# GLAD-RUC/FastEGNN

Measured on AMD Instinct MI355X. Metric: graphs/sec (fwd+bwd), Water-3D-like 100k-node frame, higher is better.
Workload: dtype f32; 1 GPU; cfg4 Water-3D-like frame (SURVEY 8d): uniform points, radius graph r=0.035 (mean degree ~19), gravity on; 4-layer FastEGNN H=64, fwd+loss+bwd, CSR build inside the step; nodes=100000, edges=1919172, graphs_per_batch=1, virtual_channels=16, layers=4, parallelism=1 GPU, launch=whole step replayed as one captured HIP graph

## Files before the change

### fastegnn_amd/csrc/layer_bwd.hip

```cpp
#include "stages.h"
#ifdef FE_DIAG_NOSTORE
#define WG_STORE(x)
#else
#define WG_STORE(x) x
#endif

namespace fe {

__device__ __forceinline__ Vec vdsilu_mul(const Vec &g, const Vec &z FE_ACT_P) {
  return vmap2(g, z, [=](float a, float b) { return a * dsilu_f(b FE_ACT_A); });
}
__device__ __forceinline__ Vec vmask(const Vec &v, bool keep) { return keep ? v : vzero(); }

__device__ __forceinline__ void vec_reduce_lds(float *red_row, const Vec &acc, int j, int q) {
#pragma unroll
  for (int t = 0; t < 4; ++t)
#pragma unroll
    for (int r = 0; r < 4; ++r) {
      float s = jsum(acc.t[t][r]);
      if (j == 0) atomicAdd(&red_row[16 * t + 4 * q + r], s);
    }
}

struct GraphPostBwdArgs {
  const float *xsum, *HvT, *poolV, *g_Z_out, *g_HvT_out, *wpack, *b5;
  float *g_Z, *g_HvT, *g_poolV, *g_poolX, *wg_u, *wg_gz5, *wg_pm;
  int B, C, flags;
  float act_param = 0.f;
};
__global__ __launch_bounds__(256) void graph_post_bwd_kernel(GraphPostBwdArgs a) {
  const bool bf = a.flags & FASTEGNN_F_BF16;
  auto rb = [&](const Vec &v) { return bf ? vround(v) : v; };
  const int l = lane_id(), j = l & 15, q = l >> 4;
  const int wave = global_wave_id(), nwaves = (gridDim.x * blockDim.x) >> 6;
  const int M = a.B * a.C, ntiles = (M + 15) >> 4;
  for (int i = blockIdx.x * blockDim.x + threadIdx.x; i < a.B * 3 * a.C; i += gridDim.x * blockDim.x) {
    const int b = i / (3 * a.C);
    const float g = a.g_Z_out[i];
    a.g_Z[i] = g;
    a.g_poolX[i] = g / fmaxf(a.xsum[b * 4 + 3], 1.f);
  }
  if (a.flags & FASTEGNN_F_RF) {
    for (int i = blockIdx.x * blockDim.x + threadIdx.x; i < M * H; i += gridDim.x * blockDim.x) {
      a.g_HvT[i] = a.g_HvT_out[i];
      a.g_poolV[i] = 0.f;
    }
    return;
  }
  for (int tile = wave; tile < ntiles; tile += nwaves) {
    const int m = tile * 16 + j;
    const bool valid = m < M;
    const int mc = valid ? m : M - 1;
    const int b = mc / a.C;
    const float inv = 1.0f / fmaxf(a.xsum[b * 4 + 3], 1.f);
    const Vec hv = vload_row(a.HvT + (size_t)mc * H, q);
    const Vec pm = vscale(vload_row(a.poolV + (size_t)mc * H, q), inv);
    Vec z5 = vload_vec(a.b5, q);
    gemm64(a.wpack + (size_t)I_W5A * IMG, rb(hv), z5);
    gemm64(a.wpack + (size_t)I_W5B * IMG, rb(pm), z5);
    const Vec g_out = vload_row(a.g_HvT_out + (size_t)mc * H, q);
    Vec g_u = vzero();
    gemm64(a.wpack + (size_t)I_W6T * IMG, rb(g_out), g_u);
    const Vec g_z5 = vdsilu_mul(g_u, z5 FE_ACT(a));
    Vec g_hv = (a.flags & FASTEGNN_F_RESIDUAL) ? g_out : vzero();
    gemm64(a.wpack + (size_t)I_W5AT * IMG, rb(g_z5), g_hv);
    Vec g_pm = vzero();
    gemm64(a.wpack + (size_t)I_W5BT * IMG, rb(g_z5), g_pm);
    if (valid) {
      vstore_row(a.wg_u + (size_t)m * H, q, vsilu(z5 FE_ACT(a)));
      vstore_row(a.wg_gz5 + (size_t)m * H, q, g_z5);
      vstore_row(a.wg_pm + (size_t)m * H, q, pm);
      vstore_row(a.g_HvT + (size_t)m * H, q, g_hv);
      vstore_row(a.g_poolV + (size_t)m * H, q, vscale(g_pm, inv));
    }
  }
}

int graph_post_backward(const fastegnn_layer_t *L, hipStream_t st, WgradBatch *shared) {
  FE_REQUIRE(L->xsum && L->HvT && L->poolV && L->g_Z_out && L->g_HvT_out && L->g_Z && L->g_HvT && L->g_poolV &&
                 L->g_poolX && L->wg_node && L->grads && L->wpack,
             "graph_post_backward: null buffer");
  const long M = (long)L->B * L->C;
  float *wg_gp = L->wg_node + 4 * wg_node_rows(L) * H;
  float *wg_u = wg_gp, *wg_gz5 = wg_gp + M * H, *wg_pm = wg_gp + 2 * M * H;
  GraphPostBwdArgs a{L->xsum, L->HvT, L->poolV, L->g_Z_out, L->g_HvT_out, L->wpack, L->params[FASTEGNN_P_NODEV0_B],
                     L->g_Z, L->g_HvT, L->g_poolV, L->g_poolX, wg_u, wg_gz5, wg_pm, L->B, L->C, L->flags, L->act_param};
  int grid = cdiv(cdiv(M, 16), 4);
  if (grid > 256) grid = 256;
  if (grid < 1) grid = 1;
  { ProfScope _ps_graph_post_bwd_kernel(K_GRAPH_POST_BWD, st); hipLaunchKernelGGL(graph_post_bwd_kernel, dim3(grid), dim3(256), 0, st, a); }
  int rc = check_launch("graph_post_bwd_kernel");
  if (rc) return rc;
  if (has(L, FASTEGNN_F_RF)) return FASTEGNN_OK;
  float *const *g = L->grads;
  WgradBatch local(L->wg_slab, st);
  WgradBatch &wb = shared ? *shared : local;
  wb.round = has(L, FASTEGNN_F_BF16);
  if ((rc = wb.add(L->g_HvT_out, H, wg_u, H, M, g[FASTEGNN_P_NODEV2_W], H, 0, 1, g[FASTEGNN_P_NODEV2_B]))) return rc;
  if ((rc = wb.add(wg_gz5, H, L->HvT, H, M, g[FASTEGNN_P_NODEV0_W], 2 * H, 0, 1, g[FASTEGNN_P_NODEV0_B]))) return rc;
  if ((rc = wb.add(wg_gz5, H, wg_pm, H, M, g[FASTEGNN_P_NODEV0_W], 2 * H, H, 1, nullptr))) return rc;
  return shared ? FASTEGNN_OK : wb.finish();
}


struct GraphPreBwdArgs {
  const float *xsum, *Z, *g_Bc, *g_Zp, *V0W;
  float *g_Z, *g_HvT, *g_xbar, *wg_mxt;
  int B, C, bf16;
};
constexpr int GPB_SPLIT = 4;
__global__ __launch_bounds__(256) void graph_pre_bwd_kernel(GraphPreBwdArgs a) {
  extern __shared__ float sm[];
  const int C = a.C, b = blockIdx.x, ld = 2 * H + 1 + C;
  const int i0 = blockIdx.y * 256 + threadIdx.x, istep = 256 * gridDim.y;
  float *mz = sm;
  float *gmX = sm + 3 * C;
  float *gmz = gmX + C * C;
  const float cnt = fmaxf(a.xsum[b * 4 + 3], 1.f);
  for (int i = threadIdx.x; i < 3 * C; i += 256) mz[i] = a.Z[(size_t)b * 3 * C + i] - a.xsum[b * 4 + i / C] / cnt;
  __syncthreads();
  for (int i = i0; i < C * H; i += istep) {
    int c = i >> 6, d = i & 63;
    float v = 0.f;
    if (d < C) v = mz[c] * mz[d] + mz[C + c] * mz[C + d] + mz[2 * C + c] * mz[2 * C + d];
    a.wg_mxt[((size_t)b * C + c) * H + d] = v;
  }
  for (int i = i0; i < C * H; i += istep) {
    int c = i >> 6, k = i & 63;
    const float *gb = a.g_Bc + ((size_t)b * C + c) * H;
    float acc = 0.f;
    if (a.bf16) { for (int o = 0; o < H; ++o) acc += round_bf(gb[o]) * round_bf(a.V0W[(size_t)o * ld + H + k]); }
    else { for (int o = 0; o < H; ++o) acc += gb[o] * a.V0W[(size_t)o * ld + H + k]; }
    a.g_HvT[((size_t)b * C + c) * H + k] += acc;
  }
  for (int i = threadIdx.x; i < C * C; i += 256) {
    int cp = i / C, c = i % C;
    const float *gb = a.g_Bc + ((size_t)b * C + c) * H;
    float acc = 0.f;
    for (int o = 0; o < H; ++o) acc += gb[o] * a.V0W[(size_t)o * ld + 2 * H + 1 + cp];
    gmX[cp * C + c] = acc;
  }
  __syncthreads();
  for (int i = threadIdx.x; i < 3 * C; i += 256) {
    int k = i / C, c = i % C;
    float acc = 0.f;
    for (int d = 0; d < C; ++d) acc += (gmX[c * C + d] + gmX[d * C + c]) * mz[k * C + d];
    gmz[i] = acc;
    if (i % gridDim.y == blockIdx.y) a.g_Z[(size_t)b * 3 * C + i] += acc + a.g_Zp[(size_t)b * 3 * C + i];
  }
  __syncthreads();
  if (threadIdx.x < 3 && blockIdx.y == 0) {
    float acc = 0.f;
    for (int c = 0; c < C; ++c) acc += gmz[threadIdx.x * C + c];
    a.g_xbar[b * 3 + threadIdx.x] = -acc / cnt;
  }
}
int graph_pre_backward(const fastegnn_layer_t *L, hipStream_t st, WgradBatch *shared) {
  FE_REQUIRE(L->xsum && L->Z && L->HvT && L->g_Bc && L->g_Zp && L->g_Z && L->g_HvT && L->g_xbar && L->wg_node && L->grads,
             "graph_pre_backward: null buffer");
  const long M = (long)L->B * L->C;
  float *wg_mxt = L->wg_node + 7 * wg_node_rows(L) * H;
  GraphPreBwdArgs a{L->xsum, L->Z, L->g_Bc, L->g_Zp, L->params[FASTEGNN_P_VIRT0_W], L->g_Z, L->g_HvT, L->g_xbar, wg_mxt,
                    L->B, L->C, has(L, FASTEGNN_F_BF16) ? 1 : 0};
  const size_t lds = (size_t)(6 * L->C + L->C * L->C) * sizeof(float);
  { ProfScope _ps_graph_pre_bwd_kernel(K_GRAPH_PRE_BWD, st); hipLaunchKernelGGL(graph_pre_bwd_kernel, dim3(L->B, GPB_SPLIT), dim3(256), lds, st, a); }
  int rc = check_launch("graph_pre_bwd_kernel");
  if (rc) return rc;
  float *const *g = L->grads;
  const int ld = 2 * H + 1 + L->C;
  WgradBatch local(L->wg_slab, st);
  WgradBatch &wb = shared ? *shared : local;
  wb.round = has(L, FASTEGNN_F_BF16);
  if ((rc = wb.add(L->g_Bc, H, L->HvT, H, M, g[FASTEGNN_P_VIRT0_W], ld, H, 1, g[FASTEGNN_P_VIRT0_B]))) return rc;
  wb.round = false;
  if ((rc = wb.add(L->g_Bc, H, wg_mxt, H, M, g[FASTEGNN_P_VIRT0_W], ld, 2 * H + 1, 1, nullptr, 1, 0, 0, 0, L->C))) return rc;
  return shared ? FASTEGNN_OK : wb.finish();
}

struct EdgeBwdArgs {
  EdgeArgs f;
  const float *g_aggm, *g_aggx;
  float *g_P, *g_xrow, *g_QXe;
  float *g_QXs_atomic;
  float *g_ea;
  float *d_wx2, *d_attw, *d_attb, *d_bx2;
  float *d_wr, *d_we;
  int ld_e0, C;
  float *slab, *slab_b;
  int slab_w2, slab_wx1;
  float *cons_scratch;
};
#ifndef FE_PC_PRIO
#define FE_PC_PRIO 3
#endif

#ifndef FE_PC_WAVES
#define FE_PC_WAVES 8
#endif
constexpr int PC_WAVES = FE_PC_WAVES;
constexpr int PC_CONS = 3, PC_CONS2 = 7;
constexpr int PC_PROD = PC_WAVES - 2;
#ifndef FE_PC_CONS32
#define FE_PC_CONS32 1
#endif
#ifndef FE_PC_RING
#define FE_PC_RING 3
#endif
constexpr int PC_RING = FE_PC_RING;
#ifndef FE_PC_FLUSH
#define FE_PC_FLUSH 48
#endif
constexpr int PC_FLUSH = FE_PC_FLUSH;
constexpr int PC_RS = 68;
constexpr int PC_SLOT = 2 * 16 * PC_RS;
template <int MODE> constexpr int pc_img_floats() { return 2 * (rm_lds_bytes<MODE>() / 4); }
enum { PC_HEAD = 0, PC_TOTAL = 2, PC_FILLED = 4, PC_DRAINED = 4 + 2 * PC_RING, PC_CTRL = 4 + 4 * PC_RING };
#ifdef FE_SAFE_WAITS
__device__ __forceinline__ int lds_ld(const int *p) { return __hip_atomic_load(p, __ATOMIC_ACQUIRE, __HIP_MEMORY_SCOPE_WORKGROUP); }
__device__ __forceinline__ void lds_st(int *p, int v) { __hip_atomic_store(p, v, __ATOMIC_RELEASE, __HIP_MEMORY_SCOPE_WORKGROUP); }
#else
__device__ __forceinline__ int lds_ld(const int *p) { return __atomic_load_n(p, __ATOMIC_RELAXED); }
__device__ __forceinline__ void lds_st(int *p, int v) { __atomic_store_n(p, v, __ATOMIC_RELAXED); }
#endif
__device__ __forceinline__ void pc_tile_store(float *tile, int j, int q, const Vec &v) {
#pragma unroll
  for (int t = 0; t < 4; ++t) *reinterpret_cast<f32x4 *>(tile + j * PC_RS + 16 * t + 4 * q) = v.t[t];
}
template <int MODE, int EA>
__global__ __launch_bounds__(64 * PC_WAVES) void edge_bwd_pc_kernel(EdgeBwdArgs A) {
  extern __shared__ __attribute__((aligned(16))) float lds[];
#ifdef FE_ISA_CONST
// ... 784 lines not shown
```

### fastegnn_amd/csrc/layer_fwd.hip

```cpp
#include <cstdlib>
#include "stages.h"

namespace fe {

struct NodePreArgs {
  const float *h, *x, *wpack;
  const float *b1, *bv0, *wv2, *bv2, *bg0, *wg2, *bg2;
  float *P, *QX, *A, *svel, *sgrav;
  int N, gravity, has_vel;
  const float *vel, *wv0;
  int C;
  int flags = 0;
  float act_param = 0.f;
};

template <int MODE>
__global__ __launch_bounds__(64 * NODE_PRE_WAVES) void node_pre_fwd_kernel(NodePreArgs a) {
  extern __shared__ __attribute__((aligned(16))) float lds[];
  unsigned *img = reinterpret_cast<unsigned *>(lds);
  float *vec = lds + 5 * IMG3;
  const int nimg = a.gravity ? 5 : 4;
  load_images_x3(img, wpack_x3(a.wpack, a.C, I_W1A), nimg);
  if constexpr (edge_fold_first<MODE>()) { for (int i = threadIdx.x; i < H; i += blockDim.x) vec[i] = a.b1 ? a.b1[i] * LOG2E_F : 0.f; }
  else load_floats(vec + 0 * H, a.b1, H);
// ... 174 lines not shown
    if (a.bf16) { for (int k = 0; k < H; ++k) acc += round_bf(w[H + k]) * round_bf(hv[k]); }
    else { for (int k = 0; k < H; ++k) acc += w[H + k] * hv[k]; }
    for (int d = 0; d < C; ++d) acc += w[2 * H + 1 + d] * mX[d * C + c];
    a.Bc[((size_t)b * C + c) * H + o] = acc;
  }
}
int graph_pre_forward(const fastegnn_layer_t *L, hipStream_t st) {
  FE_REQUIRE(L->xsum && L->Z && L->HvT && L->Bc, "graph_pre_forward: null buffer");
  GraphPreArgs a{L->xsum, L->Z, L->HvT, L->params[FASTEGNN_P_VIRT0_W], L->params[FASTEGNN_P_VIRT0_B], L->Bc, L->B, L->C,
                 has(L, FASTEGNN_F_BF16) ? 1 : 0};
  const size_t lds = (size_t)(3 * L->C + L->C * L->C) * sizeof(float);
  { ProfScope _ps_graph_pre_fwd_kernel(K_GRAPH_PRE_FWD, st); hipLaunchKernelGGL(graph_pre_fwd_kernel, dim3(L->B, GP_SPLIT), dim3(256), lds, st, a); }
  return check_launch("graph_pre_fwd_kernel");
}

constexpr int EDGE_FWD_IMG_FLOATS = 2 * IMG3;
template <int MODE>
__global__ __launch_bounds__(64 * EDGE_FWD_WAVES) void edge_fwd_kernel(EdgeArgs a, int C) {
  extern __shared__ __attribute__((aligned(16))) float lds[];
#ifdef FE_ISA_CONST
  a.flags = FE_ISA_CONST; a.ea_dim = 2; a.bx2 = nullptr; a.attw = nullptr;
#endif
  float *img = lds;
  float *vec = lds + EDGE_FWD_IMG_FLOATS;
  float *tiles = vec + EV_COUNT * H;
  load_images_x3(reinterpret_cast<unsigned *>(img), wpack_x3(a.wpack, C, I_W2), 2);
  constexpr bool FOLD = edge_fold<false, MODE, false>();
  edge_load_vecs(vec, a, FOLD);
  __syncthreads();
  const int l = lane_id(), j = l & 15, q = l >> 4, wv = wave_id();
  float *mt = tiles + wv * (16 * TS + 64);
  float *xt = mt + 16 * TS;
  const int wave = global_wave_id(), nwaves = (gridDim.x * blockDim.x) >> 6;
  const bool mean = !(a.flags & FASTEGNN_F_COORDS_SUM);
  FE_T0()
  const int c0 = (int)((long)wave * a.n_chunks / nwaves), c1 = (int)((long)(wave + 1) * a.n_chunks / nwaves);
  {
    const int r0 = a.chunk_row[c0], r1 = a.chunk_row[c1];
    if (r0 < r1) {
      const int e0 = a.rowptr[r0], e1 = a.rowptr[r1];
      int cur = -1;
      float acc = 0.f, accx = 0.f;
      FE_T(7)
      int cnt = 0;
      auto flush = [&]() {
        const float inv = rcp_f((float)cnt);
        a.aggm[(size_t)cur * H + l] = acc * (FOLD ? inv * LN2_F : inv);
        if (l < 3) a.aggx[(size_t)cur * 3 + l] = mean ? accx * inv : accx;
      };
      auto zero_rows = [&](int ra, int rb) {
        for (int r = ra; r < rb; ++r) {
          a.aggm[(size_t)r * H + l] = 0.f;
          if (l < 3) a.aggx[(size_t)r * 3 + l] = 0.f;
        }
      };
      EdgeIdx cur_i, nxt_i;
      if (e0 < e1) edge_load_idx(a, min(e0 + j, e1 - 1), cur_i);
      for (int base = e0; base < e1; base += 16) {
        const int nvalid = min(16, e1 - base);
        nxt_i = cur_i;
        if (base + 16 < e1) edge_load_idx(a, min(base + 16 + j, e1 - 1), nxt_i);
        EdgeFwdState S;
        Vec pre;
        edge_tile_forward<false, MODE>(a, img, vec, cur_i, q, S, pre FE_TA);
        cur_i = nxt_i;
        tile_store(mt, j, q, S.m);
        if (q == 0) {
          xt[j * 4 + 0] = S.dn[0] * S.s;
          xt[j * 4 + 1] = S.dn[1] * S.s;
          xt[j * 4 + 2] = S.dn[2] * S.s;
        }
        __builtin_amdgcn_wave_barrier();
        FE_T(5)
        float mv[16], xv[16];
#pragma unroll
        for (int ee = 0; ee < 16; ++ee) {
          mv[ee] = mt[ee * TS + l];
          xv[ee] = xt[ee * 4 + (l & 3)];
        }
        const int rowv = S.row;
#ifndef FE_WALK_READLANE
        const int prevrow = __builtin_amdgcn_update_dpp(rowv, rowv, 0x111, 0xf, 0xf, false);
        const unsigned long long chg = __builtin_amdgcn_ballot_w64(j == 0 ? rowv != cur : rowv != prevrow);
        const unsigned starts = (unsigned)chg & 0xffffu;
#endif
#pragma unroll
        for (int ee = 0; ee < 16; ++ee) {
          if (ee < nvalid) {
#ifndef FE_WALK_READLANE
            if ((starts >> ee) & 1u) {
              const int rw = __builtin_amdgcn_readlane(rowv, ee);
#else
            const int rw = __builtin_amdgcn_readlane(rowv, ee);
            if (rw != cur) {
#endif
              if (cur >= 0) flush();
              zero_rows(cur >= 0 ? cur + 1 : r0, rw);
              cur = rw;
              acc = 0.f;
              accx = 0.f;
              cnt = 0;
            }
            acc += mv[ee];
            accx += xv[ee];
            ++cnt;
          }
        }
        __builtin_amdgcn_wave_barrier();
        FE_T(6)
      }
      if (cur >= 0) flush();
      zero_rows(cur >= 0 ? cur + 1 : r0, r1);
    }
  }
  FE_TEND()
}

int edge_forward(const fastegnn_layer_t *L, hipStream_t st) {
  FE_REQUIRE(L->P && L->QX && L->aggm && L->aggx && L->wpack, "edge_forward: null buffer");
  FE_REQUIRE(L->ea <= 7, "edge_forward: edge_attr_nf > 7 unsupported");
  FE_REQUIRE(!has(L, FASTEGNN_F_ATTENTION) || (L->params[FASTEGNN_P_ATT_W] && L->params[FASTEGNN_P_ATT_B]),
             "edge_forward: attention params null");
  const fastegnn_graph_t &g = L->graph;
  if (g.n_edges == 0 || L->N == 0) {
    (void)hipMemsetAsync(L->aggm, 0, (size_t)L->N * H * sizeof(float), st);
    (void)hipMemsetAsync(L->aggx, 0, (size_t)L->N * 3 * sizeof(float), st);
    return check_launch("edge_forward(memset)");
  }
  FE_REQUIRE(g.rowptr && g.erow && g.col && g.chunk_row && (L->ea == 0 || L->ea_sorted), "edge_forward: null graph");
  EdgeArgs a = make_edge_args(L);
  FE_REQUIRE((size_t)L->N * QXLD < (1u << 30) && (size_t)g.n_src * QXLD < (1u << 30) && (size_t)g.n_edges * 8 < (1u << 30),
             "edge_forward: tables exceed the 32-bit offset range of the gather path");
#if FE_EDGE_FWD32
  if (edge_forward32_applies(L)) return edge_forward32(L, st);
#endif
  int grid = cdiv(g.n_chunks, EDGE_FWD_WAVES);
  if (grid > 256) grid = 256;
  const size_t lds = (EDGE_FWD_IMG_FLOATS + EV_COUNT * H + EDGE_FWD_WAVES * (16 * TS + 64)) * sizeof(float);
  {
    ProfScope _ps_edge_fwd_kernel(K_EDGE_FWD, st);
    if (has(L, FASTEGNN_F_BF16)) hipLaunchKernelGGL(edge_fwd_kernel<GM_BF16>, dim3(grid), dim3(64 * EDGE_FWD_WAVES), lds, st, a, L->C);
    else hipLaunchKernelGGL(edge_fwd_kernel<GM_EDGE_FWD>, dim3(grid), dim3(64 * EDGE_FWD_WAVES), lds, st, a, L->C);
  }
  return check_launch("edge_fwd_kernel");
}


}
#include "virt_fwd.h"
namespace fe {

int virt_forward(const fastegnn_layer_t *L, hipStream_t st) {
  const bool egnn = has(L, FASTEGNN_F_EGNN);
  FE_REQUIRE(L->h && L->A && L->x && L->vel && L->aggm && L->aggx && L->svel && L->npre && L->h_out && L->x_out &&
                 L->batch && L->wpack,
             "virt_forward: null buffer");
  FE_REQUIRE(egnn ? L->C == 0 : (L->Bc && L->Z && L->poolV && L->poolX && L->C >= 1 && L->C <= 64),
             "virt_forward: virtual_channels must be in [1,64] (0 with FASTEGNN_F_EGNN) and the virtual buffers non-null");
  FE_REQUIRE(L->na == 0 || L->node_attr, "virt_forward: node_attr null");
  if (L->C > 0) {
    (void)hipMemsetAsync(L->poolV, 0, (size_t)L->B * L->C * H * sizeof(float), st);
    (void)hipMemsetAsync(L->poolX, 0, (size_t)L->B * 3 * L->C * sizeof(float), st);
  }
  if (L->N == 0) return check_launch("virt_forward(memset)");
  VirtArgs a = make_virt_args(L);
  static const bool pair_off = getenv("FASTEGNN_VIRT_FWD_PAIR") && atoi(getenv("FASTEGNN_VIRT_FWD_PAIR")) == 0;
  const bool pair = GM_VIRT_FWD == GM_F16 && !pair_off && !has(L, FASTEGNN_F_BF16) && !has(L, FASTEGNN_F_RF) && !egnn && L->C >= 2 &&
                    cdiv(L->N, 16 * (VIRT_WAVES / 2)) <= 256 && virt_fwd_lds_bytes(L->C, true) <= 160 * 1024;
  const int ntg = cdiv(L->N, 16 * (pair ? VIRT_WAVES / 2 : VIRT_WAVES));
  int grid = ntg < 256 ? ntg : 256;
  {
    ProfScope _ps_virt_fwd_kernel(K_VIRT_FWD, st);
    const size_t lds = virt_fwd_lds_bytes(L->C, pair);
    if (has(L, FASTEGNN_F_BF16)) hipLaunchKernelGGL(virt_fwd_kernel<GM_BF16>, dim3(grid), dim3(64 * VIRT_WAVES), lds, st, a);
    else if (pair) launch_virt_fwd_pair(a, grid, lds, st);
    else hipLaunchKernelGGL(virt_fwd_kernel<GM_VIRT_FWD>, dim3(grid), dim3(64 * VIRT_WAVES), lds, st, a);
  }
  return check_launch("virt_fwd_kernel");
}

struct GraphPostArgs {
  const float *xsum, *Z, *HvT, *poolV, *poolX, *wpack, *b5, *b6;
  float *Z_out, *HvT_out;
  int B, C, flags;
  float act_param = 0.f;
};
__global__ __launch_bounds__(256) void graph_post_fwd_kernel(GraphPostArgs a) {
  const bool bf = a.flags & FASTEGNN_F_BF16;
  const int l = lane_id(), j = l & 15, q = l >> 4;
  const int wave = global_wave_id(), nwaves = (gridDim.x * blockDim.x) >> 6;
  const int M = a.B * a.C, ntiles = (M + 15) >> 4;
  for (int i = blockIdx.x * blockDim.x + threadIdx.x; i < a.B * 3 * a.C; i += gridDim.x * blockDim.x) {
    const int b = i / (3 * a.C);
    a.Z_out[i] = a.Z[i] + a.poolX[i] / fmaxf(a.xsum[b * 4 + 3], 1.f);
  }
  if (a.flags & FASTEGNN_F_RF) {
    for (int i = blockIdx.x * blockDim.x + threadIdx.x; i < M * H; i += gridDim.x * blockDim.x) a.HvT_out[i] = a.HvT[i];
    return;
  }
  for (int tile = wave; tile < ntiles; tile += nwaves) {
    const int m = tile * 16 + j;
    const bool valid = m < M;
    const int mc = valid ? m : M - 1;
    const int b = mc / a.C;
    const float inv = 1.0f / fmaxf(a.xsum[b * 4 + 3], 1.f);
    const Vec hv = vload_row(a.HvT + (size_t)mc * H, q);
    const Vec pm = vscale(vload_row(a.poolV + (size_t)mc * H, q), inv);
    Vec z5 = vload_vec(a.b5, q);
    gemm64(a.wpack + (size_t)I_W5A * IMG, bf ? vround(hv) : hv, z5);
    gemm64(a.wpack + (size_t)I_W5B * IMG, bf ? vround(pm) : pm, z5);
    Vec out = vload_vec(a.b6, q);
    const Vec u5 = vsilu(z5 FE_ACT(a));
    gemm64(a.wpack + (size_t)I_W6 * IMG, bf ? vround(u5) : u5, out);
    if (a.flags & FASTEGNN_F_RESIDUAL) vadd(out, hv);
    if (valid) vstore_row(a.HvT_out + (size_t)m * H, q, out);
  }
}
int graph_post_forward(const fastegnn_layer_t *L, hipStream_t st) {
  FE_REQUIRE(L->xsum && L->Z && L->HvT && L->poolV && L->poolX && L->Z_out && L->HvT_out && L->wpack,
             "graph_post_forward: null buffer");
  GraphPostArgs a{L->xsum, L->Z, L->HvT, L->poolV, L->poolX, L->wpack, L->params[FASTEGNN_P_NODEV0_B],
                  L->params[FASTEGNN_P_NODEV2_B], L->Z_out, L->HvT_out, L->B, L->C, L->flags, L->act_param};
  int grid = cdiv(cdiv((long)L->B * L->C, 16), 4);
  if (grid > 256) grid = 256;
  if (grid < 1) grid = 1;
  { ProfScope _ps_graph_post_fwd_kernel(K_GRAPH_POST_FWD, st); hipLaunchKernelGGL(graph_post_fwd_kernel, dim3(grid), dim3(256), 0, st, a); }
  return check_launch("graph_post_fwd_kernel");
}

}

#ifdef FE_STAMP_VF
extern "C" int fastegnn_debug_read_stamps_vf(unsigned long long *out, int reset) {
  if (hipMemcpyFromSymbol(out, HIP_SYMBOL(fe::g_vf_stamps), sizeof(unsigned long long) * 16) != hipSuccess) return -1;
  if (reset) {
    unsigned long long z[16] = {0};
    (void)hipMemcpyToSymbol(HIP_SYMBOL(fe::g_vf_stamps), z, sizeof(z));
  }
  return 0;
}
#endif
#ifdef FE_STAMP
extern "C" int fastegnn_debug_read_stamps(unsigned long long *out, int reset) {
  if (hipMemcpyFromSymbol(out, HIP_SYMBOL(fe::g_stamps), sizeof(unsigned long long) * 16) != hipSuccess) return -1;
  if (reset) {
    unsigned long long z[16] = {0};
    (void)hipMemcpyToSymbol(HIP_SYMBOL(fe::g_stamps), z, sizeof(z));
  }
  return 0;
}
#endif
```

### fastegnn_amd/csrc/stages.h

```cpp
#pragma once
#include "kernels.h"

namespace fe {

#ifndef FE_EDGE_FWD_WAVES
#define FE_EDGE_FWD_WAVES 16
#endif
constexpr int EDGE_FWD_WAVES = FE_EDGE_FWD_WAVES;
#ifndef FE_NODE_PRE_WAVES
#define FE_NODE_PRE_WAVES 8
#endif
constexpr int NODE_PRE_WAVES = FE_NODE_PRE_WAVES;
#ifndef FE_VIRT_WAVES
#define FE_VIRT_WAVES 8
#endif
constexpr int VIRT_WAVES = FE_VIRT_WAVES;
#ifndef FE_VIRT_BWD_WAVES
#define FE_VIRT_BWD_WAVES 4
#endif
constexpr int VIRT_BWD_WAVES = FE_VIRT_BWD_WAVES;

struct EdgeArgs {
  const float *P, *QX, *QXs, *ea, *wpack;
  const float *E0W, *b2, *bx1, *wx2, *attw, *attb, *bx2;
// ... 177 lines not shown
  gemm_e<MODE, 0, RM>(img, S.t, S.mp);
  FE_T(3)
  if constexpr (FOLD) S.m0 = vsilu2(S.mp);
  else S.m0 = KEEP_D ? vsilu_keep_d(S.mp FE_ACT(a)) : vsilu(S.mp FE_ACT(a));
  if (a.flags & FASTEGNN_F_ATTENTION) {
    S.att = sigmoid_f(vdot(S.m0, vload_vec(vec + EV_ATT * H, q)) + a.attb[0]);
    S.m = vscale(S.m0, S.att);
  } else {
    S.att = 1.f;
    S.m = S.m0;
  }
  FE_T(2)
  S.up = vload_vec(vec + EV_BX1 * H, q);
  gemm_e<MODE, 1, RM>(img, S.m, S.up);
  FE_T(3)
  if constexpr (FOLD) S.u = vsilu2(S.up);
  else S.u = KEEP_D ? vsilu_keep_d(S.up FE_ACT(a)) : vsilu(S.up FE_ACT(a));
  const float sraw = vdot(S.u, vload_vec(vec + EV_WX2 * H, q)) + (a.bx2 ? a.bx2[0] : 0.f);
  S.s = (a.flags & FASTEGNN_F_TANH) ? tanh_f(sraw) : sraw;
  FE_T(4)
}
template <bool KEEP_D, int MODE = GM_F32, bool RM = false>
__device__ __forceinline__ void edge_tile_forward(const EdgeArgs &a, const void *img, const float *vec,
                                                  const EdgeIdx &I, int q, EdgeFwdState &S, Vec &pre FE_TP) {
  EdgeRows G;
  edge_gather(a, I, q, G);
  edge_tile_pre<edge_fold_first<MODE>()>(a, vec, I, G, q, S, pre FE_TA);
  edge_tile_mlp<KEEP_D, MODE, RM>(a, img, vec, q, S, pre FE_TA);
}

inline EdgeArgs make_edge_args(const fastegnn_layer_t *L) {
  const float *const *p = L->params;
  const fastegnn_graph_t &g = L->graph;
  EdgeArgs a{L->P, L->QX, L->QX_src ? L->QX_src : L->QX, L->ea_sorted, L->wpack,
             p[FASTEGNN_P_EDGE0_W], p[FASTEGNN_P_EDGE2_B], p[FASTEGNN_P_CR0_B], p[FASTEGNN_P_CR2_W],
             p[FASTEGNN_P_ATT_W], p[FASTEGNN_P_ATT_B], p[FASTEGNN_P_CR2_B], g.rowptr, g.erow, g.col, g.chunk_row, L->aggm, L->aggx,
             g.n_chunks, L->ea, L->flags, L->epsilon};
  a.act_param = L->act_param;
  return a;
}

struct VirtArgs {
  const float *h, *A, *Bc, *x, *vel, *Z, *aggm, *aggx, *svel, *sgrav, *node_attr, *wpack;
  const float *V0W, *c2, *bxv0, *wxv2, *bxx0, *wxx2, *attw, *attb, *N0W, *b3, *b4;
  const int32_t *batch;
  float *h_out, *x_out, *npre, *poolV, *poolX;
  int N, B, C, na, flags;
  float g[3];
  float act_param = 0.f;
};
constexpr int VV_WVR = 0, VV_C2 = 1, VV_BXV0 = 2, VV_WXV2 = 3, VV_BXX0 = 4, VV_WXX2 = 5, VV_ATT = 6, VV_B3 = 7,
              VV_B4 = 8, VV_COUNT = 9;

template <int MODE>
struct VirtFwdState {
  Vec pre, t, vp, v0, v, uxp, uXp;
  typename OperandOf<MODE>::type vs;
  float vd[3], vr, att, sx, sX;
};

__device__ __forceinline__ void virt_load_vecs(float *vec, const VirtArgs &a) {
  const int ld = 2 * H + 1 + a.C;
  for (int i = threadIdx.x; i < H; i += blockDim.x) {
    vec[VV_WVR * H + i] = a.V0W ? a.V0W[(size_t)i * ld + 2 * H] : 0.f;
    vec[VV_C2 * H + i] = a.c2 ? a.c2[i] : 0.f;
    vec[VV_BXV0 * H + i] = a.bxv0 ? a.bxv0[i] : 0.f;
    vec[VV_WXV2 * H + i] = a.wxv2 ? a.wxv2[i] : 0.f;
    vec[VV_BXX0 * H + i] = a.bxx0 ? a.bxx0[i] : 0.f;
    vec[VV_WXX2 * H + i] = a.wxx2 ? a.wxx2[i] : 0.f;
    vec[VV_ATT * H + i] = a.attw ? a.attw[i] : 0.f;
    vec[VV_B3 * H + i] = a.b3 ? a.b3[i] : 0.f;
    vec[VV_B4 * H + i] = a.b4 ? a.b4[i] : 0.f;
  }
}

template <int MODE = GM_F32>
__device__ __forceinline__ void virt_tile_forward(const VirtArgs &a, const void *img, const float *vec, const Vec &Ai,
                                                  const float xi[3], int b, int c, int q, const float *BcL,
                                                  const float *ZL, VirtFwdState<MODE> &S VF_TP) {
  const int C = a.C;
  if (ZL) {
    S.vd[0] = ZL[c] - xi[0];
    S.vd[1] = ZL[C + c] - xi[1];
    S.vd[2] = ZL[2 * C + c] - xi[2];
  } else {
    const float *Zb = a.Z + (size_t)b * 3 * C;
    S.vd[0] = Zb[c] - xi[0];
    S.vd[1] = Zb[C + c] - xi[1];
    S.vd[2] = Zb[2 * C + c] - xi[2];
  }
  S.vr = sqrt_f(S.vd[0] * S.vd[0] + S.vd[1] * S.vd[1] + S.vd[2] * S.vd[2]);
#ifdef FE_VIRT_PRE_MFMA
  if (BcL) {
    const int j = lane_id() & 15;
    const float *wsrc = (q == 0 ? vec + VV_WVR * H : BcL + c * H) + j;
    const float f = q == 0 ? S.vr : (q == 1 ? 1.f : 0.f);
#pragma unroll
    for (int t = 0; t < 4; ++t) S.pre.t[t] = __builtin_amdgcn_mfma_f32_16x16x4f32(wsrc[16 * t], f, Ai.t[t], 0, 0, 0);
  } else
#endif
  {
    S.pre = Ai;
    if (BcL) vadd(S.pre, vload_vec(BcL + c * H, q));
    else vadd(S.pre, vload_row(a.Bc + ((size_t)b * C + c) * H, q));
    vaxpy(S.pre, S.vr, vload_vec(vec + VV_WVR * H, q));
  }
  S.t = vsilu(S.pre FE_ACT(a));
  VF_T(1)
  S.vp = vload_vec(vec + VV_C2 * H, q);
  VF_PRIO_ON();
  gemm_i<MODE>(img, 0, S.t, S.vp);
  VF_PRIO_OFF();
  VF_T(2)
  S.v0 = vsilu(S.vp FE_ACT(a));
  if (a.flags & FASTEGNN_F_ATTENTION) {
    S.att = sigmoid_f(vdot(S.v0, vload_vec(vec + VV_ATT * H, q)) + a.attb[0]);
    S.v = vscale(S.v0, S.att);
  } else {
    S.att = 1.f;
    S.v = S.v0;
  }
  S.uxp = vload_vec(vec + VV_BXV0 * H, q);
  S.vs = make_operand<MODE>(S.v);
  VF_T(3)
  VF_PRIO_ON();
  gemm_op<MODE>(img, 1, S.vs, S.uxp);
  VF_PRIO_OFF();
  VF_T(4)
  float sr = vdot(vsilu(S.uxp FE_ACT(a)), vload_vec(vec + VV_WXV2 * H, q));
  S.sx = (a.flags & FASTEGNN_F_TANH) ? tanh_f(sr) : sr;
  VF_T(5)
  S.uXp = vload_vec(vec + VV_BXX0 * H, q);
  VF_PRIO_ON();
  gemm_op<MODE>(img, 2, S.vs, S.uXp);
  VF_PRIO_OFF();
  VF_T(4)
  sr = vdot(vsilu(S.uXp FE_ACT(a)), vload_vec(vec + VV_WXX2 * H, q));
  S.sX = (a.flags & FASTEGNN_F_TANH) ? tanh_f(sr) : sr;
  VF_T(5)
}

inline VirtArgs make_virt_args(const fastegnn_layer_t *L) {
  const float *const *p = L->params;
  VirtArgs a{L->h, L->A, L->Bc, L->x, L->vel, L->Z, L->aggm, L->aggx, L->svel, L->sgrav, L->node_attr, L->wpack,
             p[FASTEGNN_P_VIRT0_W], p[FASTEGNN_P_VIRT2_B], p[FASTEGNN_P_CRV0_B], p[FASTEGNN_P_CRV2_W],
             p[FASTEGNN_P_CVV0_B], p[FASTEGNN_P_CVV2_W], p[FASTEGNN_P_ATTV_W], p[FASTEGNN_P_ATTV_B],
             p[FASTEGNN_P_NODE0_W], p[FASTEGNN_P_NODE0_B], p[FASTEGNN_P_NODE2_B], L->batch,
             L->h_out, L->x_out, L->npre, L->poolV, L->poolX, L->N, L->B, L->C, L->na, L->flags,
             {L->gravity[0], L->gravity[1], L->gravity[2]}};
  a.act_param = L->act_param;
  return a;
}
void launch_virt_fwd_pair(const VirtArgs &a, int grid, size_t lds, hipStream_t st);
inline size_t virt_lds_bytes(int C, int n_img, int waves = VIRT_WAVES) {
  return (size_t)(n_img * IMG + 16 * H + waves * 16 * TS + C * H + 4 * C) * sizeof(float);
}


}
```

### fastegnn_amd/csrc/virt_bwd.hip

```cpp
#include <cstdlib>
#include "stages.h"

namespace fe {

#ifdef FE_SAFE_WAITS
__device__ __forceinline__ int vb_ld(const int *p) { return __hip_atomic_load(p, __ATOMIC_ACQUIRE, __HIP_MEMORY_SCOPE_WORKGROUP); }
__device__ __forceinline__ void vb_st(int *p, int v) { __hip_atomic_store(p, v, __ATOMIC_RELEASE, __HIP_MEMORY_SCOPE_WORKGROUP); }
#else
__device__ __forceinline__ int vb_ld(const int *p) { return __atomic_load_n(p, __ATOMIC_RELAXED); }
__device__ __forceinline__ void vb_st(int *p, int v) { __atomic_store_n(p, v, __ATOMIC_RELAXED); }
#endif

#ifdef FE_STAMP
__device__ unsigned long long g_vb2_stamps[32];
#define VB2_T0() unsigned _vp = (unsigned)__builtin_amdgcn_s_memtime(); unsigned _va[12] = {0, 0, 0, 0, 0, 0, 0, 0, 0, 0, 0, 0};
#define VB2_T(i) { __builtin_amdgcn_sched_barrier(0); const unsigned _t = (unsigned)__builtin_amdgcn_s_memtime(); \
                   _va[i] += _t - _vp; _vp = _t; __builtin_amdgcn_sched_barrier(0); }
#define VB2_TEND(base) if (lane_id() == 0) { for (int _k = 0; _k < 12; ++_k) atomicAdd(&g_vb2_stamps[(base) + _k], (unsigned long long)_va[_k]); }
#elif defined(FE_ISA_MARK)
#define VB2_T0()
#define VB2_T(i) { __builtin_amdgcn_sched_barrier(0); asm volatile("; FE_MARK " #i); __builtin_amdgcn_sched_barrier(0); }
#define VB2_TEND(base)
#else
#define VB2_T0()
#define VB2_T(i)
#define VB2_TEND(base)
#endif

__device__ __forceinline__ Vec vb_dsilu_mul(const Vec &g, const Vec &z FE_ACT_P) {
  return vmap2(g, z, [=](float a, float b) { return a * dsilu_f(b FE_ACT_A); });
}
__device__ __forceinline__ Vec vb_mask(const Vec &v, bool keep) { return keep ? v : vzero(); }

struct VirtNodeArgs {
  const float *g_h_out, *npre, *g_x_out, *vel, *aggx, *wpack;
  float *wg_t3, *wg_gnp, *g_h, *g_aggm, *g_aggx, *g_svel, *g_sgrav;
  int N, flags, C;
  float g[3];
  float act_param = 0.f;
};
constexpr int VB_NODE_WAVES = 8;
template <bool BF>
__global__ __launch_bounds__(64 * VB_NODE_WAVES) void virt_bwd_node_kernel(VirtNodeArgs a) {
  constexpr int SM = BF ? GM_BF16 : GM_X3;
  extern __shared__ __attribute__((aligned(16))) float lds[];
  unsigned *img = reinterpret_cast<unsigned *>(lds);
  const bool rf = a.flags & FASTEGNN_F_RF;
  if (!rf) load_images_x3(img, wpack_x3(a.wpack, a.C, I_W3AT), 3);
  __syncthreads();
  const int l = lane_id(), j = l & 15, q = l >> 4;
  const int wave = global_wave_id(), nwaves = (gridDim.x * blockDim.x) >> 6;
  const int ntiles = (a.N + 15) >> 4;
  const bool clamp_aggx = a.flags & FASTEGNN_F_EGNN;
  for (int tile = wave; tile < ntiles; tile += nwaves) {
    const int n = tile * 16 + j;
    const bool valid = n < a.N;
    const int nc = valid ? n : a.N - 1;
    const Vec g_out = vb_mask(vload_row(a.g_h_out + (size_t)nc * H, q), valid);
    if (rf) {
      if (valid) {
        vstore_row(a.g_h + (size_t)n * H, q, g_out);
        vstore_row(a.g_aggm + (size_t)n * H, q, vzero());
      }
    } else {
      const Vec npre = vload_row(a.npre + (size_t)nc * H, q);
      Vec g_t3 = vzero();
      gemm_op<SM>(img, 2, make_operand<SM>(g_out), g_t3);
      const Vec g_np = vb_dsilu_mul(g_t3, npre FE_ACT(a));
      if (valid) {
        vstore_row(a.wg_t3 + (size_t)n * H, q, vsilu(npre FE_ACT(a)));
        vstore_row(a.wg_gnp + (size_t)n * H, q, g_np);
      }
      const typename OperandOf<SM>::type gop = make_operand<SM>(g_np);
      Vec g_h = (a.flags & FASTEGNN_F_RESIDUAL) ? g_out : vzero();
      gemm_op<SM>(img, 0, gop, g_h);
      if (valid) vstore_row(a.g_h + (size_t)n * H, q, g_h);
      Vec g_am = vzero();
      gemm_op<SM>(img, 1, gop, g_am);
      if (valid) vstore_row(a.g_aggm + (size_t)n * H, q, g_am);
    }
    if (valid && q == 0) {
      float sv = 0.f, sg = 0.f;
#pragma unroll
      for (int k = 0; k < 3; ++k) {
        const float gxn = a.g_x_out[(size_t)n * 3 + k];
        const bool pass = !clamp_aggx || fabsf(a.aggx[(size_t)n * 3 + k]) <= 100.f;
        a.g_aggx[(size_t)n * 3 + k] = pass ? gxn : 0.f;
        sv += gxn * a.vel[(size_t)n * 3 + k];
        sg += gxn * a.g[k];
      }
      a.g_svel[n] = sv;
      if (a.flags & FASTEGNN_F_GRAVITY) a.g_sgrav[n] = sg;
    }
  }
}

struct VirtGvArgs {
  const float *g_np, *g_poolV, *wpack;
  const int32_t *batch;
  float *Gv;
  size_t cstride;
  int N, C, ngroups, nranges;
};
constexpr int VB_GV_CH = 4;
constexpr int VB_GV_WAVES = 8;
template <bool BF>
__global__ __launch_bounds__(64 * VB_GV_WAVES) void virt_bwd_gv_kernel(VirtGvArgs a) {
  constexpr int SM = BF ? GM_BF16 : GM_X3;
  extern __shared__ __attribute__((aligned(16))) float lds[];
  char *img = reinterpret_cast<char *>(lds);
  const int grp = (int)blockIdx.x % a.ngroups, range = (int)blockIdx.x / a.ngroups;
  const int c0 = grp * VB_GV_CH, ncv = min(VB_GV_CH, a.C - c0);
  {
    const u32x4 *src = reinterpret_cast<const u32x4 *>(wpack_rm(a.wpack, a.C, RM_FIXED + c0));
    u32x4 *dst = reinterpret_cast<u32x4 *>(img);
    for (int i = threadIdx.x; i < ncv * (RM_BYTES / 16); i += blockDim.x) dst[i] = src[i];
  }
  __syncthreads();
  const int l = lane_id(), j = l & 15, q = l >> 4, wv = wave_id();
  const int ntiles = (a.N + 15) >> 4;
  const int t_lo = (int)((long)range * ntiles / a.nranges), t_hi = (int)((long)(range + 1) * ntiles / a.nranges);
  for (int tile = t_lo + wv; tile < t_hi; tile += VB_GV_WAVES) {
    const int n = tile * 16 + j;
    const bool valid = n < a.N;
    const int nc = valid ? n : a.N - 1;
    const int b = a.batch[nc];
    Vec g = vb_mask(vload_row(a.g_np + (size_t)nc * H, q), valid);
    if constexpr (BF) g = vround(g);
    const typename OperandOf<SM>::type op = make_operand<SM>(g);
    const float *pv = a.g_poolV + ((size_t)b * a.C + c0) * H;
#pragma unroll 1
    for (int k = 0; k < ncv; ++k) {
      Vec acc = vload_row(pv + (size_t)k * H, q);
      gemm_rm<SM, true>(img + k * RM_BYTES, op, acc);
#ifdef VB_GV_NT
      if (valid) {
        float *row = a.Gv + (size_t)(c0 + k) * a.cstride + (size_t)n * H;
#pragma unroll
        for (int t = 0; t < 4; ++t) __builtin_nontemporal_store(acc.t[t], reinterpret_cast<f32x4 *>(row + 16 * t + 4 * q));
      }
#else
      if (valid) vstore_row(a.Gv + (size_t)(c0 + k) * a.cstride + (size_t)n * H, q, acc);
#endif
    }
  }
}

#ifndef FE_VB_FLUSH
#define FE_VB_FLUSH 48
#endif
constexpr int VB_FLUSH = FE_VB_FLUSH;
constexpr int VB_FINE_TILES = 3;
constexpr int VB_GF = 2;
constexpr int VB_WAVES = 8;
constexpr int VB_CONS_X = 3, VB_CONS_XX = 7, VB_CONS_V2 = 6;
#ifndef FE_VB_CONS32
#define FE_VB_CONS32 1
#endif
#ifndef FE_VB_6P
#define FE_VB_6P 1
#endif
constexpr int VB_RS = 68;
constexpr int VB_TILE = 16 * VB_RS;
constexpr int VB_SLOT_A = 3 * VB_TILE;
constexpr int VB_SLOT_B = 2 * VB_TILE;
constexpr int VB_MAXRING = 6;
enum { VBC_UNIT = 0, VBC_HEAD = 1, VBC_FILLED = 4, VBC_DRAINED = 4 + 2 * VB_MAXRING, VBC_CTRL = 4 + 5 * VB_MAXRING };
constexpr int VB_RACC = 5 * H;
constexpr int VB_MAXBANK = 5;

struct VirtBwd2Args {
  VirtArgs f;
  const float *g_x_out, *g_poolX, *Gv;
  float *g_x, *g_A, *g_Bc, *g_Zp;
  float *gA_part, *gx_part;
  float *wg_v;
  float *cons_scratch;
  size_t cstride;
  float *d_wxv2, *d_wxx2, *d_wvr, *d_attw, *d_attb;
  int ld_v0;
  float *slab, *slab_b;
  int slab_x, slab_X, slab_v2;
  int NGF, ringA, ringB, nbank;
};

inline size_t vb_lds_floats(int C, int ringA, int ringB, int nbank, int img_bytes = RM_BYTES) {
  return (size_t)3 * (img_bytes / 4) + VV_COUNT * H + (size_t)nbank * VB_RACC + (size_t)C * H + ((3 * C + 3) & ~3) + (size_t)ringA * VB_SLOT_A +
         (size_t)ringB * VB_SLOT_B + VBC_CTRL;
}

__device__ __forceinline__ void vb_tile_store(float *tile, int j, int q, const Vec &v) {
#pragma unroll
  for (int t = 0; t < 4; ++t) *reinterpret_cast<f32x4 *>(tile + j * VB_RS + 16 * t + 4 * q) = v.t[t];
}
__device__ __forceinline__ void vb_accum_items(float *row, const Vec &u, int j, int q) {
#ifdef VB_DIAG_NOACC
  if (u.t[0][0] == 12345.678f) row[0] = 1.f;
  return;
#endif
  tile_sum_add(row, u, j, q);
}

template <bool BF, bool ATT>
__global__ __launch_bounds__(64 * VB_WAVES) void virt_bwd_pc_kernel(VirtBwd2Args A) {
  constexpr int SM = BF ? GM_BF16 : GM_VIRT_BWD;
  typedef typename OperandOf<SM>::type SOp;
  extern __shared__ __attribute__((aligned(16))) float lds[];
  const VirtArgs &a = A.f;
  const int C = a.C;
  constexpr int RMS = rm_lds_bytes<SM>();
  char *rmimg = reinterpret_cast<char *>(lds);
  float *vec = lds + 3 * (RMS / 4);
  float *racc0 = vec + VV_COUNT * H;
  float *gBc_l = racc0 + A.nbank * VB_RACC;
  float *gZ_l = gBc_l + C * H;
  float *ringA = gZ_l + ((3 * C + 3) & ~3);
  float *ringB = ringA + A.ringA * VB_SLOT_A;
  int *ctrl = reinterpret_cast<int *>(ringB + A.ringB * VB_SLOT_B);
  {
    const char *src = wpack_rm(a.wpack, C, SM == GM_F16 ? RM_F16 : 0);
    for (int i = threadIdx.x; i < 3 * (RMS / 16); i += blockDim.x) {
      const int im = i / (RMS / 16), k = i % (RMS / 16);
      reinterpret_cast<u32x4 *>(rmimg + im * RMS)[k] = reinterpret_cast<const u32x4 *>(src + (size_t)im * RM_BYTES)[k];
    }
  }
  virt_load_vecs(vec, a);
  for (int i = threadIdx.x; i < A.nbank * VB_RACC + C * H + 3 * C; i += blockDim.x) racc0[i] = 0.f;
  if (threadIdx.x < VBC_CTRL) ctrl[threadIdx.x] = 0;
  __syncthreads();
  const int l = lane_id(), j = l & 15, q = l >> 4, wv = wave_id();
  constexpr bool CONS32 = SM == GM_F16 && FE_VB_CONS32 != 0;
  constexpr bool SIXP = CONS32 && FE_VB_6P != 0;
  const bool consumer = wv == VB_CONS_X || wv == VB_CONS_XX || (!SIXP && wv == VB_CONS_V2);
  const int ntiles = (a.N + 15) >> 4;
  const int t_lo = (int)((long)blockIdx.x * ntiles / gridDim.x), t_hi = (int)((long)(blockIdx.x + 1) * ntiles / gridDim.x);
  const int n_fine = min(t_hi - t_lo, VB_FINE_TILES), n_coarse = t_hi - t_lo - n_fine;
  const int n_units = n_coarse + n_fine * A.NGF;
#ifdef VB_DIAG_NOPUB
  const int total = 0;
#else
  const int total = (t_hi - t_lo) * C;
#endif
  const int cur = a.batch[t_lo * 16];
  const bool tanh_on = a.flags & FASTEGNN_F_TANH;

  if (CONS32 && consumer) {
    if constexpr (CONS32) {
    __builtin_amdgcn_s_setprio(3);
    const bool ringA_wave = SIXP ? wv == VB_CONS_X : wv != VB_CONS_V2;
// ... 446 lines not shown
          float pz[3];
#pragma unroll
          for (int k = 0; k < 3; ++k) pz[k] = jsum((valid && q == 0) ? g_vd[k] : 0.f);
          vb_accum_items(pmode == 0 ? gBc_l + c * H : A.g_Bc + ((size_t)b0 * C + c) * H, g_pre, j, q);
          if (l < 3) {
            const float pzl = l == 0 ? pz[0] : (l == 1 ? pz[1] : pz[2]);
            if (pmode == 0) atomicAdd(&gZ_l[l * C + c], pzl);
            else atomicAdd(&A.g_Zp[((size_t)b0 * 3 + l) * C + c], pzl);
          }
        } else {
          if (valid && q == 0) {
#pragma unroll
            for (int k = 0; k < 3; ++k) atomicAdd(&A.g_Zp[((size_t)b * 3 + k) * C + c], g_vd[k]);
          }
          if (valid) {
#pragma unroll
            for (int t2 = 0; t2 < 4; ++t2)
#pragma unroll
              for (int r = 0; r < 4; ++r)
                atomicAdd(&A.g_Bc[((size_t)b * C + c) * H + 16 * t2 + 4 * q + r], g_pre.t[t2][r]);
          }
        }
        VB2_T(10)
      }
      if (valid && q == 0) {
        if (grp == 0) {
#pragma unroll
          for (int k = 0; k < 3; ++k) A.g_x[(size_t)n * 3 + k] = gx[k];
        } else {
          *reinterpret_cast<f32x4 *>(A.gx_part + (part * 16 + j) * 4) = f32x4{gx[0], gx[1], gx[2], 0.f};
        }
      }
    }
    VB2_TEND(0)
  }
  VB2_T0()
  __syncthreads();
  VB2_T(11)
  VB2_TEND(consumer ? 12 : 0)
  for (int i = threadIdx.x; i < C * H; i += blockDim.x) atomicAdd(&A.g_Bc[(size_t)cur * C * H + i], gBc_l[i]);
  for (int i = threadIdx.x; i < 3 * C; i += blockDim.x) atomicAdd(&A.g_Zp[(size_t)cur * 3 * C + i], gZ_l[i]);
  if (threadIdx.x < H) {
    const int o = threadIdx.x;
    float s5[5] = {0.f, 0.f, 0.f, 0.f, 0.f};
    for (int bk = 0; bk < A.nbank; ++bk) {
      const float *r = racc0 + bk * VB_RACC;
#pragma unroll
      for (int k = 0; k < 4; ++k) s5[k] += r[k * H + o];
      s5[4] += r[4 * H];
    }
    atomicAdd(&A.d_wxv2[o], s5[0]);
    atomicAdd(&A.d_wxx2[o], s5[1]);
    atomicAdd(&A.d_wvr[(size_t)o * A.ld_v0], s5[2]);
    if constexpr (ATT) {
      atomicAdd(&A.d_attw[o], s5[3]);
      if (o == 0) atomicAdd(A.d_attb, s5[4]);
    }
  }
}

__global__ __launch_bounds__(256) void virt_bwd_combine_kernel(float *g_A, float *g_x, const float *gA_part, const float *gx_part,
                                                               int N, int nparts, int grid_pc) {
  const int wg = (int)blockIdx.x / VB_FINE_TILES, fslot = (int)blockIdx.x % VB_FINE_TILES;
  const int ntiles = (N + 15) >> 4;
  const int t_lo = (int)((long)wg * ntiles / grid_pc), t_hi = (int)((long)(wg + 1) * ntiles / grid_pc);
  const int n_fine = min(t_hi - t_lo, VB_FINE_TILES);
  if (fslot >= n_fine) return;
  const int tile = t_hi - n_fine + fslot;
  const size_t p0 = (size_t)blockIdx.x * nparts;
  const int row = threadIdx.x >> 4, c4 = threadIdx.x & 15;
  const int n = tile * 16 + row;
  if (n >= N) return;
  f32x4 s = reinterpret_cast<const f32x4 *>(g_A + (size_t)n * H)[c4];
  for (int p = 0; p < nparts; ++p) s += reinterpret_cast<const f32x4 *>(gA_part + ((p0 + p) * 16 + row) * H)[c4];
  reinterpret_cast<f32x4 *>(g_A + (size_t)n * H)[c4] = s;
  if (c4 < 3) {
    float sx = g_x[(size_t)n * 3 + c4];
    for (int p = 0; p < nparts; ++p) sx += gx_part[((p0 + p) * 16 + row) * 4 + c4];
    g_x[(size_t)n * 3 + c4] = sx;
  }
}

#ifndef FE_VB_CS
#define FE_VB_CS 1
#endif
#ifndef FE_VBS_5P
#define FE_VBS_5P 1
#endif
constexpr int VBS_SLOT_A = 4 * VB_TILE;
constexpr int VBS_W3_WORDS = 4096;
constexpr int VBS_MIN_TILES = 12;
constexpr int VBS_MAXC = 64;
constexpr int VBS_MAXTILES = 256;
#ifndef FE_VBS_BLOCK
#define FE_VBS_BLOCK 24
#endif
constexpr int VBS_BLOCK = FE_VBS_BLOCK;
constexpr int VBS_NPH = 64;
enum { VBSC_UNIT = 0, VBSC_HEAD = 1, VBSC_FILLED = 4, VBSC_DRAINED = 4 + 2 * VB_MAXRING, VBSC_SLOTCH = 4 + 5 * VB_MAXRING,
       VBSC_READY = 4 + 6 * VB_MAXRING, VBSC_DONE = 4 + 6 * VB_MAXRING + VBS_NPH, VBSC_TSEQ = 4 + 6 * VB_MAXRING + 2 * VBS_NPH,
       VBSC_CTRL = 4 + 6 * VB_MAXRING + 2 * VBS_NPH + VBS_MAXTILES };

struct VirtCsArgs {
  VirtArgs f;
  const float *g_x_out, *g_poolX, *g_poolV, *g_np;
  float *g_x, *g_A, *g_Bc, *g_Zp;
  float *cons_scratch;
  float *w_slab;
  float *d_wxv2, *d_wxx2, *d_wvr, *d_attw, *d_attb;
  int ld_v0;
  float *slab, *slab_b;
  int slab_x, slab_X, slab_v2;
  int ringA, ringB, nbank;
  int block;
};
inline size_t vbs_lds_floats(int ringA, int ringB, int nbank) {
  return (size_t)3 * (rm_lds_bytes<GM_F16>() / 4) + 2 * VBS_W3_WORDS + VV_COUNT * H + (size_t)nbank * VB_RACC + 2 * H + 8 +
         (size_t)ringA * VBS_SLOT_A + (size_t)ringB * VB_SLOT_B + VBSC_CTRL;
}

__device__ __forceinline__ void gemm64_f2_scaled(const unsigned *img3, const Split2s &in, Vec &acc) {
  const u32x4 *ip = reinterpret_cast<const u32x4 *>(img3) + lane_id();
  const f16x8 xh0 = __builtin_bit_cast(f16x8, in.s.p[0][0]), xh1 = __builtin_bit_cast(f16x8, in.s.p[0][1]);
  const f16x8 xl0 = __builtin_bit_cast(f16x8, in.s.p[1][0]), xl1 = __builtin_bit_cast(f16x8, in.s.p[1][1]);
#pragma unroll
  for (int t = 0; t < 4; ++t) {
    const f16x8 ah0 = __builtin_bit_cast(f16x8, ip[(t * 2 + 0) * 64]), ah1 = __builtin_bit_cast(f16x8, ip[(t * 2 + 1) * 64]);
    const f16x8 al0 = __builtin_bit_cast(f16x8, ip[512 + (t * 2 + 0) * 64]), al1 = __builtin_bit_cast(f16x8, ip[512 + (t * 2 + 1) * 64]);
    f32x4 lo = {0.f, 0.f, 0.f, 0.f};
    lo = __builtin_amdgcn_mfma_f32_16x16x32_f16(al0, xh0, lo, 0, 0, 0);
    lo = __builtin_amdgcn_mfma_f32_16x16x32_f16(ah0, xl0, lo, 0, 0, 0);
    lo = __builtin_amdgcn_mfma_f32_16x16x32_f16(al1, xh1, lo, 0, 0, 0);
    lo = __builtin_amdgcn_mfma_f32_16x16x32_f16(ah1, xl1, lo, 0, 0, 0);
    f32x4 hi;
#pragma unroll
    for (int r = 0; r < 4; ++r) hi[r] = lo[r] * F2_DOWN;
    hi = __builtin_amdgcn_mfma_f32_16x16x32_f16(ah0, xh0, hi, 0, 0, 0);
    hi = __builtin_amdgcn_mfma_f32_16x16x32_f16(ah1, xh1, hi, 0, 0, 0);
#pragma unroll
    for (int r = 0; r < 4; ++r) acc.t[t][r] = __builtin_fmaf(hi[r], in.inv, acc.t[t][r]);
  }
}

#ifdef FE_VBS_WATCHDOG
__device__ int g_vbs_dog[64];
#define VBS_SPIN(id, cond, sl) { long _n = 0; while (cond) { __builtin_amdgcn_s_sleep(sl); if (++_n > 3000000) { if (lane_id() == 0) { atomicAdd(&g_vbs_dog[id], 1); if (blockIdx.x == 0 && g_vbs_dog[48 + wave_id()] == 0) g_vbs_dog[48 + wave_id()] = (id) * 1000000 + _mark; } break; } } }
#define VBS_MARK(x) _mark = (x)
#else
#define VBS_SPIN(id, cond, sl) { int _n = 0; while (cond) { __builtin_amdgcn_s_sleep(sl); if (++_n > VBS_SPIN_LIMIT) { if (lane_id() == 0) atomicAdd(&g_vbs_timeouts, 1); break; } } }
#define VBS_MARK(x)
#endif
constexpr int VBS_SPIN_LIMIT = 1 << 23;
__device__ int g_vbs_timeouts = 0;
template <bool ATT>
__global__ __launch_bounds__(64 * VB_WAVES) void virt_bwd_cs_kernel(VirtCsArgs A) {
  constexpr int SM = GM_F16;
  typedef typename OperandOf<SM>::type SOp;
  extern __shared__ __attribute__((aligned(16))) float lds[];
#ifdef FE_VBS_WATCHDOG
  int _mark = 0;
#endif
#ifdef FE_ISA_CONST
  A.f.flags = FE_ISA_CONST; A.f.B = 1;
#endif
  const VirtArgs &a = A.f;
  const int C = a.C;
  constexpr int RMS = rm_lds_bytes<SM>();
  char *rmimg = reinterpret_cast<char *>(lds);
  unsigned *w3 = reinterpret_cast<unsigned *>(lds) + 3 * (RMS / 4);
  float *vec = lds + 3 * (RMS / 4) + 2 * VBS_W3_WORDS;
  float *racc0 = vec + VV_COUNT * H;
  float *gBc_l = racc0 + A.nbank * VB_RACC;
  float *gZ_l = gBc_l + 2 * H;
  float *ringA = gZ_l + 8;
  float *ringB = ringA + A.ringA * VBS_SLOT_A;
  int *ctrl = reinterpret_cast<int *>(ringB + A.ringB * VB_SLOT_B);
  const int l = lane_id(), j = l & 15, q = l >> 4, wv = wave_id();
  auto stage_w3 = [&](int ph) {
    const int c = ph % C;
    const u32x4 *src = reinterpret_cast<const u32x4 *>(wpack_x3(a.wpack, C, img_w3ct(C, c)));
    u32x4 *dst = reinterpret_cast<u32x4 *>(w3 + (ph & 1) * VBS_W3_WORDS);
    u32x4 tmp[16];
#pragma unroll
    for (int i = 0; i < 16; ++i) tmp[i] = src[l + 64 * i];
#pragma unroll
    for (int i = 0; i < 16; ++i) dst[l + 64 * i] = tmp[i];
  };
  {
    const char *src = wpack_rm(a.wpack, C, RM_F16);
    for (int i = threadIdx.x; i < 3 * (RMS / 16); i += blockDim.x) {
      const int im = i / (RMS / 16), k = i % (RMS / 16);
      reinterpret_cast<u32x4 *>(rmimg + im * RMS)[k] = reinterpret_cast<const u32x4 *>(src + (size_t)im * RM_BYTES)[k];
    }
  }
  virt_load_vecs(vec, a);
  for (int i = threadIdx.x; i < A.nbank * VB_RACC + 2 * H + 8; i += blockDim.x) racc0[i] = 0.f;
  if (threadIdx.x < VBSC_CTRL) ctrl[threadIdx.x] = 0;
  const int ntiles = (a.N + 15) >> 4;
  const int t_lo = (int)((long)blockIdx.x * ntiles / gridDim.x), t_hi = (int)((long)(blockIdx.x + 1) * ntiles / gridDim.x);
  const int nt = t_hi - t_lo;
  const int nblk = max(1, (nt + A.block / 2) / A.block);
  const int BT = (nt + nblk - 1) / nblk;
  const int nphase = nblk * C;
  if (wv == 0) stage_w3(0);
  if (wv == 1 && nphase > 1) stage_w3(1);
  __syncthreads();
  if (threadIdx.x < 2 && (int)threadIdx.x < nphase) ctrl[VBSC_READY + threadIdx.x] = threadIdx.x + 1;
  __syncthreads();
  constexpr bool FIVEP = FE_VBS_5P != 0;
  const bool consumer = wv == VB_CONS_X || wv == VB_CONS_XX || (FIVEP && wv == VB_CONS_V2);
  const int total = nt * C;
  const int cur = a.batch[t_lo * 16];
  const bool tanh_on = a.flags & FASTEGNN_F_TANH;

  if (consumer) {
    __builtin_amdgcn_s_setprio(3);
    const bool wx = wv == VB_CONS_X;
    auto scp = [&](int slot, int blk, int e4) {
      char *b = reinterpret_cast<char *>(A.cons_scratch + ((size_t)blockIdx.x * 5 + slot) * IMG) + (size_t)((blk * 4 + e4) * 64 * 16);
      asm volatile("" : "+s"(b));
      return reinterpret_cast<f32x4 *>(b + (unsigned)l * 16u);
    };
    auto flush_one = [&](WgAcc32 &acc, float ig, float it, int slot, bool have, bool last, float *slab_dst) {
#pragma unroll
      for (int bo = 0; bo < 2; ++bo)
#pragma unroll
        for (int bk = 0; bk < 2; ++bk)
#pragma unroll
          for (int e4 = 0; e4 < 4; ++e4) {
            f32x4 v;
#pragma unroll
            for (int r = 0; r < 4; ++r) v[r] = (acc.c[bo][bk][4 * e4 + r] * ig) * it;
            f32x4 *d = scp(slot, bo * 2 + bk, e4);
            if (have) v += *d;
            if (!last) {
              *d = v;
            } else {
#pragma unroll
              for (int r = 0; r < 4; ++r) slab_dst[(32 * bo + 8 * e4 + 4 * (l >> 5) + r) * H + 32 * bk + (l & 31)] = v[r];
            }
#pragma unroll
            for (int r = 0; r < 4; ++r) acc.c[bo][bk][4 * e4 + r] = 0.f;
          }
    };
    auto bias_out = [&](double (&bs)[2], size_t sl) {
#pragma unroll
      for (int b = 0; b < 2; ++b) {
        double s0 = bs[b];
        s0 += __shfl_xor(s0, 32);
        if (l < 32) A.slab_b[sl * H + 32 * b + l] = (float)s0;
      }
    };
    auto rowsum8 = [](const float (&x)[2][8], int b) {
      return (double)(((x[b][0] + x[b][1]) + (x[b][2] + x[b][3])) + ((x[b][4] + x[b][5]) + (x[b][6] + x[b][7])));
    };
    WgAcc32 acc0, acc1;
    wg32_zero(acc0);
    wg32_zero(acc1);
    const int *filledA = ctrl + VBSC_FILLED, *filledB = ctrl + VBSC_FILLED + VB_MAXRING;
    if (wx) {
      WgScale sG0{0}, sG1{0}, sT{0};
      double bs0[2] = {0., 0.}, bs1[2] = {0., 0.};
      bool flushed = false;
      int since = 0;
      int *drained = ctrl + VBSC_DRAINED;
      for (int done = 0; done < total; ++done) {
        VBS_MARK(done);
        const int s0 = done % A.ringA, r0w = done / A.ringA;
        VBS_SPIN(1, vb_ld(&filledA[s0]) != r0w + 1, 1);
        __builtin_amdgcn_fence(__ATOMIC_ACQUIRE, "workgroup", "local");
        const float *g0 = ringA + s0 * VBS_SLOT_A;
        float xt[2][8], xg0[2][8], xg1[2][8];
        wg32_read<VB_RS>(g0 + 2 * VB_TILE, xt);
        wg32_read<VB_RS>(g0, xg0);
        wg32_read<VB_RS>(g0 + VB_TILE, xg1);
        __builtin_amdgcn_fence(__ATOMIC_RELEASE, "workgroup", "local");
        __builtin_amdgcn_s_waitcnt(0xc07f);
        if (l == 0) vb_st(&drained[s0], r0w + 1);
        const float fT = sT.update_lazy(xt);
        const float f0 = sG0.update_lazy(xg0) * fT, f1 = sG1.update_lazy(xg1) * fT;
        if (f0 != 1.f) wg32_scale_acc(acc0, f0);
        if (f1 != 1.f) wg32_scale_acc(acc1, f1);
        const WgOp32 T = wg32_split(xt, sT.scale());
        {
          const WgOp32 G = wg32_split(xg0, sG0.scale());
          bs0[0] += rowsum8(xg0, 0); bs0[1] += rowsum8(xg0, 1);
          wg32_mma(acc0, G, T);
        }
        {
          const WgOp32 G = wg32_split(xg1, sG1.scale());
          bs1[0] += rowsum8(xg1, 0); bs1[1] += rowsum8(xg1, 1);
          wg32_mma(acc1, G, T);
        }
        if (++since >= VB_FLUSH && done + 1 < total) {
          flush_one(acc0, sG0.inv(), sT.inv(), 0, flushed, false, nullptr);
          flush_one(acc1, sG1.inv(), sT.inv(), 1, flushed, false, nullptr);
          flushed = true;
          since = 0;
        }
      }
      const size_t slx = (size_t)A.slab_x + blockIdx.x, slX = (size_t)A.slab_X + blockIdx.x;
      flush_one(acc0, sG0.inv(), sT.inv(), 0, flushed, true, A.slab + slx * IMG);
      flush_one(acc1, sG1.inv(), sT.inv(), 1, flushed, true, A.slab + slX * IMG);
      bias_out(bs0, slx);
      bias_out(bs1, slX);
    } else {
      WgScale sGv{0}, sTv{0}, sGw{0}, sTw{0};
      double bsv[2] = {0., 0.};
      bool flushed_v = false;
      int since_v = 0, doneA = 0, doneB = 0;
      int w_ch = -1;
      int w_cnt[2] = {0, 0};
      bool w_have[2] = {false, false};
      int since_w = 0;
      int *drainedA = ctrl + VBSC_DRAINED + VB_MAXRING, *drainedB = ctrl + VBSC_DRAINED + 2 * VB_MAXRING;
#ifdef FE_VBS_SWAP
      const bool doV2 = FIVEP ? wv == VB_CONS_V2 : wv == VB_CONS_XX, doW = wv == VB_CONS_XX;
#else
      const bool doV2 = wv == VB_CONS_XX, doW = FIVEP ? wv == VB_CONS_V2 : wv == VB_CONS_XX;
#endif
      auto flush_w = [&](WgAcc32 &acc, float ig, float it, int slot, bool have, float *dst, bool add) {
#pragma unroll
        for (int bo = 0; bo < 2; ++bo)
#pragma unroll
          for (int bk = 0; bk < 2; ++bk)
#pragma unroll
            for (int e4 = 0; e4 < 4; ++e4) {
              f32x4 v;
#pragma unroll
              for (int r = 0; r < 4; ++r) v[r] = (acc.c[bo][bk][4 * e4 + r] * ig) * it;
              if (have) v += *scp(slot, bo * 2 + bk, e4);
              f32x4 *d = reinterpret_cast<f32x4 *>(dst + (size_t)(((bo * 2 + bk) * 4 + e4) * 64 * 4)) + l;
              if (add) v += *d;
              *d = v;
#pragma unroll
              for (int r = 0; r < 4; ++r) acc.c[bo][bk][4 * e4 + r] = 0.f;
            }
      };
      int w_par = 0;
      auto park_w = [&]() {
        if (w_ch < 0) return;
        flush_one(acc1, sGw.inv(), sTw.inv(), 3 + w_par, w_have[w_par], false, nullptr);
        w_have[w_par] = true;
      };
#ifdef FE_VBS_WATCHDOG
      long dog = 0;
#endif
      int idle = 0;
      while ((doW && doneA < total) || (doV2 && doneB < total)) {
        bool did = false;
        if (doV2 && doneB < total) {
          const int s0 = doneB % A.ringB, r0w = doneB / A.ringB;
          if (vb_ld(&filledB[s0]) == r0w + 1) {
            __builtin_amdgcn_fence(__ATOMIC_ACQUIRE, "workgroup", "local");
            const float *g0 = ringB + s0 * VB_SLOT_B;
            float xg[2][8], xt[2][8];
            wg32_read<VB_RS>(g0, xg);
            wg32_read<VB_RS>(g0 + VB_TILE, xt);
            __builtin_amdgcn_fence(__ATOMIC_RELEASE, "workgroup", "local");
            __builtin_amdgcn_s_waitcnt(0xc07f);
            if (l == 0) vb_st(&drainedB[s0], r0w + 1);
            const float f = sGv.update_lazy(xg) * sTv.update_lazy(xt);
            if (f != 1.f) wg32_scale_acc(acc0, f);
            const WgOp32 G = wg32_split(xg, sGv.scale()), T = wg32_split(xt, sTv.scale());
            bsv[0] += rowsum8(xg, 0); bsv[1] += rowsum8(xg, 1);
            wg32_mma(acc0, G, T);
            ++doneB;
            if (++since_v >= VB_FLUSH && doneB < total) {
              flush_one(acc0, sGv.inv(), sTv.inv(), 2, flushed_v, false, nullptr);
              flushed_v = true;
              since_v = 0;
            }
            did = true;
          }
        }
        if (doW && doneA < total) {
          const int s0 = doneA % A.ringA, r0w = doneA / A.ringA;
          if (vb_ld(&filledA[s0]) == r0w + 1) {
            __builtin_amdgcn_fence(__ATOMIC_ACQUIRE, "workgroup", "local");
            const float *g0 = ringA + s0 * VBS_SLOT_A;
            const int chw = __builtin_amdgcn_readfirstlane(ctrl[VBSC_SLOTCH + s0]);
            const int ch = chw & 0xff, nb_ph = (chw >> 8) & 0xfff, first_blk = chw >> 20;
            const int par = (first_blk * C + ch) & 1;
            float xg[2][8], xt[2][8];
            wg32_read<VB_RS>(g0 + 3 * VB_TILE, xg);
            wg32_read<VB_RS>(g0 + 2 * VB_TILE, xt);
            __builtin_amdgcn_fence(__ATOMIC_RELEASE, "workgroup", "local");
            __builtin_amdgcn_s_waitcnt(0xc07f);
            if (l == 0) vb_st(&drainedA[s0], r0w + 1);
            if (ch != w_ch || par != w_par) {
              park_w();
              w_ch = ch;
              w_par = par;
              since_w = 0;
            }
#ifndef VBS_DIAG_NO_W
            const float f = sGw.update_lazy(xg) * sTw.update_lazy(xt);
            if (f != 1.f) wg32_scale_acc(acc1, f);
            const WgOp32 G = wg32_split(xg, sGw.scale()), T = wg32_split(xt, sTw.scale());
            wg32_mma(acc1, G, T);
#endif
            ++doneA;
            if (++w_cnt[par] == nb_ph) {
              flush_w(acc1, sGw.inv(), sTw.inv(), 3 + par, w_have[par], A.w_slab + ((size_t)ch * gridDim.x + blockIdx.x) * IMG, first_blk != 0);
              w_have[par] = false;
              w_cnt[par] = 0;
              w_ch = -1;
            } else if (++since_w >= VB_FLUSH) {
              park_w();
              since_w = 0;
            }
            did = true;
          }
        }
        if (did) idle = 0;
        if (!did) {
          __builtin_amdgcn_s_sleep(1);
          if (++idle > VBS_SPIN_LIMIT) { if (l == 0) atomicAdd(&g_vbs_timeouts, 1); break; }
#ifdef FE_VBS_WATCHDOG
          if (++dog > 6000000) { if (l == 0) { atomicAdd(&g_vbs_dog[6], 1); if (blockIdx.x == 0) { g_vbs_dog[38] = doneA; g_vbs_dog[39] = doneB; g_vbs_dog[40] = total; g_vbs_dog[41] = ctrl[VBSC_UNIT]; g_vbs_dog[42] = ctrl[VBSC_HEAD]; g_vbs_dog[43] = ctrl[VBSC_HEAD + 1]; for (int _k = 0; _k < 8; ++_k) { g_vbs_dog[8 + _k] = ctrl[VBSC_READY + _k]; g_vbs_dog[16 + _k] = ctrl[VBSC_DONE + _k]; } } } break; }
#endif
        }
      }
      if (doV2) {
        const size_t sl = (size_t)A.slab_v2 + blockIdx.x;
        flush_one(acc0, sGv.inv(), sTv.inv(), 2, flushed_v, true, A.slab + sl * IMG);
        bias_out(bsv, sl);
      }
    }
  } else {
    const float invC = 1.0f / (float)C;
    const float attb0 = ATT ? a.attb[0] : 0.f;
    float *racc = racc0 + ((wv > 3 ? wv - 1 : wv) % A.nbank) * VB_RACC;
    auto mm = [&](int which, const SOp &op, Vec &acc) { gemm_rm<SM, false>(rmimg + which * RMS, op, acc); };
    auto mmT = [&](int which, const Vec &g, Vec &acc) {
      const auto op = make_grad_operand<SM>(g);
      gemm_rm_g<SM, true>(rmimg + which * RMS, op, acc);
    };
    int pend_tile = -1, pend_c = 0;
    VB2_T0()
    auto take = [&]() {
      int u_ = 0;
      if (l == 0) u_ = atomicAdd(&ctrl[VBSC_UNIT], 1);
      return __builtin_amdgcn_readfirstlane(u_);
    };
    auto unit_of = [&](int u_, int &blk_, int &nb_, int &c_, int &tile_) {
      const int per_blk = BT * C;
      blk_ = min(u_ / per_blk, nblk - 1);
      nb_ = min(BT, nt - blk_ * BT);
      const int ru = u_ - blk_ * per_blk;
      c_ = ru / nb_;
      tile_ = t_lo + blk_ * BT + (ru - c_ * nb_);
    };
    for (;;) {
      const int u = take();
      if (u >= total) {
        if (pend_tile >= 0) {
          __builtin_amdgcn_s_waitcnt(0x0f70);
          asm volatile("" ::: "memory");
          if (l == 0) __hip_atomic_store(&ctrl[VBSC_TSEQ + pend_tile], pend_c + 1, __ATOMIC_RELEASE, __HIP_MEMORY_SCOPE_WORKGROUP);
        }
        break;
      }
      int blk, nb, c, tile;
      unit_of(u, blk, nb, c, tile);
      const int ph = blk * C + c;
      VBS_MARK(u);
      if (pend_tile >= 0 && (vb_ld(&ctrl[VBSC_READY + ph % VBS_NPH]) != ph + 1 || vb_ld(&ctrl[VBSC_TSEQ + (tile - t_lo)]) < c)) {
        __builtin_amdgcn_s_waitcnt(0x0f70);
        asm volatile("" ::: "memory");
        if (l == 0) __hip_atomic_store(&ctrl[VBSC_TSEQ + pend_tile], pend_c + 1, __ATOMIC_RELEASE, __HIP_MEMORY_SCOPE_WORKGROUP);
        asm volatile("" ::: "memory");
        pend_tile = -1;
      }
      VBS_SPIN(2, vb_ld(&ctrl[VBSC_READY + ph % VBS_NPH]) != ph + 1, 2);
      VBS_SPIN(7, vb_ld(&ctrl[VBSC_TSEQ + (tile - t_lo)]) < c, 1);
      __builtin_amdgcn_fence(__ATOMIC_ACQUIRE, "workgroup");
      VB2_T(0)
      const int n0 = tile * 16, nend = min(a.N, n0 + 16);
      const int b0 = a.B == 1 ? 0 : a.batch[n0], b1 = a.B == 1 ? 0 : a.batch[nend - 1];
      const int pmode = b0 != b1 ? 2 : (b0 == cur ? 0 : 1);
      const int n = n0 + j;
      const bool valid = n < nend;
      const int nc = valid ? n : nend - 1;
      const int b = a.B == 1 ? 0 : a.batch[nc];
      const unsigned offB = (unsigned)b * C * H + 4u * q + (unsigned)c * H;
      const unsigned offN = (unsigned)nc * H + 4u * q;
      const unsigned offZ = (unsigned)b * 3u * C;
      float gxn[3], xi[3], gx[3];
#pragma unroll
      for (int k = 0; k < 3; ++k) {
        gxn[k] = valid ? A.g_x_out[(size_t)nc * 3 + k] : 0.f;
        xi[k] = a.x[(size_t)nc * 3 + k];
        gx[k] = c == 0 ? gxn[k] : (valid ? A.g_x[(size_t)nc * 3 + k] : 0.f);
      }
      float vd[3], gpX[3];
#pragma unroll
      for (int k = 0; k < 3; ++k) {
        vd[k] = (a.Z + (k * C + c))[offZ] - xi[k];
        gpX[k] = valid ? (A.g_poolX + (k * C + c))[offZ] : 0.f;
      }
      const float vr = sqrt_f(vd[0] * vd[0] + vd[1] * vd[1] + vd[2] * vd[2]);
      Vec vp = vload_vec(vec + VV_C2 * H, q);
      Vec d_pre = vload_u(a.A, offN);
      vadd(d_pre, vload_u(a.Bc, offB));
      vaxpy(d_pre, vr, vload_vec(vec + VV_WVR * H, q));
      const Vec t = vsilu_keep_d(d_pre FE_ACT(a));
      if (pend_tile >= 0) {
        __builtin_amdgcn_s_waitcnt(0x0f70);
        asm volatile("" ::: "memory");
        if (l == 0) __hip_atomic_store(&ctrl[VBSC_TSEQ + pend_tile], pend_c + 1, __ATOMIC_RELEASE, __HIP_MEMORY_SCOPE_WORKGROUP);
        asm volatile("" ::: "memory");
      }
      VB2_T(1)
      mm(0, make_operand<SM>(t), vp);
      VB2_T(2)
      const Vec v0 = vsilu_keep_d(vp FE_ACT(a));
      float att = 1.f;
      Vec v = v0;
      if constexpr (ATT) {
        att = sigmoid_f(vdot(v0, vload_vec(vec + VV_ATT * H, q)) + attb0);
        v = vscale(v0, att);
      }
      VB2_T(3)
      float sx, sX;
      Vec g_ux, g_uX;
      {
        Vec uxp = vload_vec(vec + VV_BXV0 * H, q), uXp = vload_vec(vec + VV_BXX0 * H, q);
        {
          const SOp vs = make_operand<SM>(v);
          mm(1, vs, uxp);
          mm(2, vs, uXp);
        }
        VB2_T(4)
        {
          Vec ux = vsilu_keep_d(uxp FE_ACT(a));
          const float sr = vdot(ux, vload_vec(vec + VV_WXV2 * H, q));
          sx = tanh_on ? tanh_f(sr) : sr;
          float g_sx = 0.f;
#pragma unroll
          for (int k = 0; k < 3; ++k) g_sx -= vd[k] * invC * gxn[k];
          const float g_sr = tanh_on ? g_sx * (1.f - sx * sx) : g_sx;
          vb_accum_items(racc + 0 * H, vscale(ux, g_sr), j, q);
          g_ux = vmul(vscale(vload_vec(vec + VV_WXV2 * H, q), g_sr), uxp);
        }
        VB2_T(5)
        {
          Vec uX = vsilu_keep_d(uXp FE_ACT(a));
          const float sr = vdot(uX, vload_vec(vec + VV_WXX2 * H, q));
          sX = tanh_on ? tanh_f(sr) : sr;
          float g_sX = 0.f;
#pragma unroll
          for (int k = 0; k < 3; ++k) g_sX += vd[k] * gpX[k];
          const float g_sr = tanh_on ? g_sX * (1.f - sX * sX) : g_sX;
          vb_accum_items(racc + 1 * H, vscale(uX, g_sr), j, q);
          g_uX = vmul(vscale(vload_vec(vec + VV_WXX2 * H, q), g_sr), uXp);
        }
      }
      VB2_T(6)
      const Vec gnp = vb_mask(vload_u(A.g_np, offN), valid);
      {
        int tk = 0;
        if (l == 0) tk = atomicAdd(&ctrl[VBSC_HEAD + 0], 1);
        tk = __builtin_amdgcn_readfirstlane(tk);
        const int sl = tk % A.ringA, round = tk / A.ringA;
        VBS_SPIN(4, vb_ld(&ctrl[VBSC_DRAINED + 0 * VB_MAXRING + sl]) != round, 2);
        VBS_SPIN(5, vb_ld(&ctrl[VBSC_DRAINED + 1 * VB_MAXRING + sl]) != round, 2);
        __builtin_amdgcn_fence(__ATOMIC_ACQUIRE, "workgroup", "local");
        float *slot = ringA + sl * VBS_SLOT_A;
        vb_tile_store(slot, j, q, g_ux);
        vb_tile_store(slot + VB_TILE, j, q, g_uX);
        vb_tile_store(slot + 2 * VB_TILE, j, q, valid ? v : vzero());
        vb_tile_store(slot + 3 * VB_TILE, j, q, gnp);
        if (l == 0) ctrl[VBSC_SLOTCH + sl] = c | (nb << 8) | (blk << 20);
        __builtin_amdgcn_fence(__ATOMIC_RELEASE, "workgroup", "local");
        if (l == 0) vb_st(&ctrl[VBSC_FILLED + sl], round + 1);
        asm volatile("" ::: "memory");
      }
      VB2_T(7)
      Vec g_v = vb_mask(vload_u(A.g_poolV, offB), valid);
      gemm64_f2_scaled(w3 + (ph & 1) * VBS_W3_WORDS, vsplit2_scaled(gnp), g_v);
      mmT(1, g_ux, g_v);
      mmT(2, g_uX, g_v);
      VB2_T(8)
      float g_vd[3];
#pragma unroll
      for (int k = 0; k < 3; ++k) g_vd[k] = -sx * invC * gxn[k] + sX * gpX[k];
      Vec g_v0 = g_v;
      if constexpr (ATT) {
        const float g_a = vdot(g_v, v0);
        const float g_z = g_a * att * (1.f - att);
        vb_accum_items(racc + 3 * H, vscale(v0, g_z), j, q);
        const float sz = jsum(q == 0 ? g_z : 0.f);
        if (l == 0) atomicAdd(&racc[4 * H], sz);
        g_v0 = vscale(g_v, att);
        vaxpy(g_v0, g_z, vload_vec(vec + VV_ATT * H, q));
      }
      Vec g_t = vzero();
      Vec ga = vzero();
      {
        const Vec g_vp = vmul(g_v0, vp);
        {
          int tk = 0;
          if (l == 0) tk = atomicAdd(&ctrl[VBSC_HEAD + 1], 1);
          tk = __builtin_amdgcn_readfirstlane(tk);
          const int sl = tk % A.ringB, round = tk / A.ringB;
          VBS_SPIN(3, vb_ld(&ctrl[VBSC_DRAINED + 2 * VB_MAXRING + sl]) != round, 2);
          __builtin_amdgcn_fence(__ATOMIC_ACQUIRE, "workgroup", "local");
          float *slot = ringB + sl * VB_SLOT_B;
          vb_tile_store(slot, j, q, g_vp);
          vb_tile_store(slot + VB_TILE, j, q, t);
          __builtin_amdgcn_fence(__ATOMIC_RELEASE, "workgroup", "local");
          if (l == 0) vb_st(&ctrl[VBSC_FILLED + VB_MAXRING + sl], round + 1);
          asm volatile("" ::: "memory");
        }
        if (c > 0) ga = vload_u(A.g_A, offN);
        mmT(0, g_vp, g_t);
      }
      VB2_T(9)
      const Vec g_pre = vmul(g_t, d_pre);
      vadd(ga, g_pre);
      if (valid) vstore_u(A.g_A, offN, ga);
      vb_accum_items(racc + 2 * H, vscale(g_pre, vr), j, q);
      const float g_vr = vdot(g_pre, vload_vec(vec + VV_WVR * H, q));
      const float ivr = vr > 0.f ? g_vr * rcp_f(vr) : 0.f;
#pragma unroll
      for (int k = 0; k < 3; ++k) {
        g_vd[k] += ivr * vd[k];
        gx[k] -= g_vd[k];
      }
      if (valid && q == 0) {
#pragma unroll
        for (int k = 0; k < 3; ++k) A.g_x[(size_t)n * 3 + k] = gx[k];
      }
      if (pmode < 2) {
        float pz[3];
#pragma unroll
        for (int k = 0; k < 3; ++k) pz[k] = jsum((valid && q == 0) ? g_vd[k] : 0.f);
        vb_accum_items(pmode == 0 ? gBc_l + (ph & 1) * H : A.g_Bc + ((size_t)b0 * C + c) * H, g_pre, j, q);
        if (l < 3) {
          const float pzl = l == 0 ? pz[0] : (l == 1 ? pz[1] : pz[2]);
          if (pmode == 0) atomicAdd(&gZ_l[(ph & 1) * 4 + l], pzl);
          else atomicAdd(&A.g_Zp[((size_t)b0 * 3 + l) * C + c], pzl);
        }
      } else {
        if (valid && q == 0) {
#pragma unroll
          for (int k = 0; k < 3; ++k) atomicAdd(&A.g_Zp[((size_t)b * 3 + k) * C + c], g_vd[k]);
        }
        if (valid) {
#pragma unroll
          for (int t2 = 0; t2 < 4; ++t2)
#pragma unroll
            for (int r = 0; r < 4; ++r)
              atomicAdd(&A.g_Bc[((size_t)b * C + c) * H + 16 * t2 + 4 * q + r], g_pre.t[t2][r]);
        }
      }
      pend_tile = tile - t_lo;
      pend_c = c;
      __builtin_amdgcn_fence(__ATOMIC_RELEASE, "workgroup", "local");
      int dn = 0;
      if (l == 0) dn = atomicAdd(&ctrl[VBSC_DONE + ph % VBS_NPH], 1);
      dn = __builtin_amdgcn_readfirstlane(dn);
      if (dn == nb - 1) {
        __builtin_amdgcn_fence(__ATOMIC_ACQUIRE, "workgroup", "local");
        const float pb = gBc_l[(ph & 1) * H + l];
        atomicAdd(&A.g_Bc[((size_t)cur * C + c) * H + l], pb);
        gBc_l[(ph & 1) * H + l] = 0.f;
        if (l < 3) {
          atomicAdd(&A.g_Zp[((size_t)cur * 3 + l) * C + c], gZ_l[(ph & 1) * 4 + l]);
          gZ_l[(ph & 1) * 4 + l] = 0.f;
        }
        if (l == 0) ctrl[VBSC_DONE + ph % VBS_NPH] = 0;
        if (ph + 2 < nphase) {
          stage_w3(ph + 2);
          asm volatile("" ::: "memory");
          if (l == 0) __hip_atomic_store(&ctrl[VBSC_READY + (ph + 2) % VBS_NPH], ph + 3, __ATOMIC_RELEASE, __HIP_MEMORY_SCOPE_WORKGROUP);
          asm volatile("" ::: "memory");
        }
      }
      VB2_T(10)
    }
    VB2_TEND(0)
  }
  VB2_T0()
  __syncthreads();
  VB2_T(11)
  VB2_TEND(consumer ? 12 : 0)
  if (threadIdx.x < H) {
    const int o = threadIdx.x;
    float s5[5] = {0.f, 0.f, 0.f, 0.f, 0.f};
    for (int bk = 0; bk < A.nbank; ++bk) {
      const float *r = racc0 + bk * VB_RACC;
#pragma unroll
      for (int k = 0; k < 4; ++k) s5[k] += r[k * H + o];
      s5[4] += r[4 * H];
    }
    atomicAdd(&A.d_wxv2[o], s5[0]);
    atomicAdd(&A.d_wxx2[o], s5[1]);
    atomicAdd(&A.d_wvr[(size_t)o * A.ld_v0], s5[2]);
    if constexpr (ATT) {
      atomicAdd(&A.d_attw[o], s5[3]);
      if (o == 0) atomicAdd(A.d_attb, s5[4]);
    }
  }
}

static int virt_cs_grid(long N) {
  const long g = ((N + 15) / 16) / VBS_MIN_TILES;
  return (int)(g > 256 ? 256 : g);
}
static int virt_cs_min_grid() {
  static const int v = getenv("FASTEGNN_VIRT_CS_MIN_GRID") ? atoi(getenv("FASTEGNN_VIRT_CS_MIN_GRID")) : 256;
  return v < 1 ? 1 : v;
}
bool virt_cs_applies(long N, int C, int flags) {
  if (!(FE_VB_CS && GM_VIRT_BWD == GM_F16 && FE_VB_CONS32)) return false;
  static const bool off = getenv("FASTEGNN_VIRT_CS") && atoi(getenv("FASTEGNN_VIRT_CS")) == 0;
  if (off || (flags & (FASTEGNN_F_BF16 | FASTEGNN_F_RF | FASTEGNN_F_EGNN)) || C < 1 || C > VBS_MAXC) return false;
  const int grid = virt_cs_grid(N);
  if (grid < 1) return false;
  static const int max_tiles = getenv("FASTEGNN_VIRT_CS_MAX_TILES") ? atoi(getenv("FASTEGNN_VIRT_CS_MAX_TILES")) : 64;
  const long nt = ((N + 15) / 16 + grid - 1) / grid;
  return grid >= virt_cs_min_grid() && nt <= VBS_MAXTILES && nt <= max_tiles;
}
size_t virt_cs_wg_floats(size_t C) { return (size_t)256 * (5 + C) * IMG; }

size_t virt_pc_wg_floats(size_t N, size_t C) {
  const size_t NGF = (C + VB_GF - 1) / VB_GF;
  return (N + WGV_PAD) * C * H + (size_t)256 * VB_FINE_TILES * (NGF - 1) * 16 * (H + 4) + (size_t)256 * 3 * IMG;
}

static int virt_backward_channels_cs(const fastegnn_layer_t *L, hipStream_t st, float *wg_gnp) {
  const int C = L->C;
  const bool att = has(L, FASTEGNN_F_ATTENTION);
  float *const *g = L->grads;
  const int grid = virt_cs_grid(L->N);
  FE_REQUIRE(L->g_poolV, "virt_backward: g_poolV null");
  WgradBatch bb(L->wg_slab, st, false, WG_SLABS / 2, WG_SLABS / 2);
  VirtCsArgs A;
  A.f = make_virt_args(L);
  A.g_x_out = L->g_x_out; A.g_poolX = L->g_poolX; A.g_poolV = L->g_poolV; A.g_np = wg_gnp;
  A.g_x = L->g_x; A.g_A = L->g_A; A.g_Bc = L->g_Bc; A.g_Zp = L->g_Zp;
  A.cons_scratch = L->wg_virt;
  A.w_slab = L->wg_virt + (size_t)grid * 5 * IMG;
  A.ld_v0 = 2 * H + 1 + C;
  A.d_wxv2 = g[FASTEGNN_P_CRV2_W]; A.d_wxx2 = g[FASTEGNN_P_CVV2_W];
  A.d_wvr = g[FASTEGNN_P_VIRT0_W] + 2 * H;
  A.d_attw = g[FASTEGNN_P_ATTV_W]; A.d_attb = g[FASTEGNN_P_ATTV_B];
  int rc;
  if ((rc = bb.add_slabs(g[FASTEGNN_P_CRV0_W], H, 0, 1, g[FASTEGNN_P_CRV0_B], grid, &A.slab_x))) return rc;
  if ((rc = bb.add_slabs(g[FASTEGNN_P_CVV0_W], H, 0, 1, g[FASTEGNN_P_CVV0_B], grid, &A.slab_X))) return rc;
  if ((rc = bb.add_slabs(g[FASTEGNN_P_VIRT2_W], H, 0, 1, g[FASTEGNN_P_VIRT2_B], grid, &A.slab_v2))) return rc;
  A.slab = bb.tab.slab; A.slab_b = bb.tab.slab_b;
  static const int ring_want = getenv("FE_VBS_RING") ? atoi(getenv("FE_VBS_RING")) : 32;
  static const int block_want = getenv("FASTEGNN_VIRT_CS_BLOCK") ? atoi(getenv("FASTEGNN_VIRT_CS_BLOCK")) : VBS_BLOCK;
  A.block = block_want < 1 ? 1 : (block_want > 0xfff ? 0xfff : block_want);
  A.ringA = ring_want / 10; A.ringB = ring_want % 10; A.nbank = 1;
  if (A.ringA < 2 || A.ringA > VB_MAXRING) A.ringA = 3;
  if (A.ringB < 2 || A.ringB > VB_MAXRING) A.ringB = 2;
  while (vbs_lds_floats(A.ringA, A.ringB, 1) * sizeof(float) > 160 * 1024 && A.ringB > 2) --A.ringB;
  while (vbs_lds_floats(A.ringA, A.ringB, 1) * sizeof(float) > 160 * 1024 && A.ringA > 2) --A.ringA;
  while (A.nbank < VB_MAXBANK && vbs_lds_floats(A.ringA, A.ringB, A.nbank + 1) * sizeof(float) <= 160 * 1024) ++A.nbank;
  const size_t lds = vbs_lds_floats(A.ringA, A.ringB, A.nbank) * sizeof(float);
  FE_REQUIRE(lds <= 160 * 1024, "virt_backward: LDS budget exceeded");
  {
    ProfScope ps(K_VIRT_BWD, st);
    const dim3 g3(grid), b3(64 * VB_WAVES);
    if (att) hipLaunchKernelGGL((virt_bwd_cs_kernel<true>), g3, b3, lds, st, A);
    else hipLaunchKernelGGL((virt_bwd_cs_kernel<false>), g3, b3, lds, st, A);
  }
  if ((rc = check_launch("virt_bwd_cs_kernel"))) return rc;
  const int ld_n0 = 2 * H + H * C + L->na;
  if ((rc = bb.add_slabs_ext(A.w_slab, g[FASTEGNN_P_NODE0_W], ld_n0, 2 * H, C, grid, C, 1))) return rc;
  return bb.finish();
}

static int virt_backward_channels(const fastegnn_layer_t *L, hipStream_t st, float *wg_gnp) {
  if (virt_cs_applies(L->N, L->C, L->flags)) return virt_backward_channels_cs(L, st, wg_gnp);
  const int N = L->N, C = L->C, ntiles = cdiv(N, 16);
  const bool bf = has(L, FASTEGNN_F_BF16), att = has(L, FASTEGNN_F_ATTENTION), rf = has(L, FASTEGNN_F_RF);
  float *const *g = L->grads;
  const size_t cstride = ((size_t)N + WGV_PAD) * H;
  float *wg_v = L->wg_virt, *Gv = L->wg_virt;
  const int NGF = (C + VB_GF - 1) / VB_GF;
  float *gA_part = Gv + cstride * C, *gx_part = gA_part + (size_t)256 * VB_FINE_TILES * (NGF - 1) * 16 * H;
  int rc;
  if (rf) {
    (void)hipMemsetAsync(Gv, 0, cstride * C * sizeof(float), st);
  } else {
    const int ngroups = cdiv(C, VB_GV_CH);
    int nranges = 256 / ngroups;
    const int max_ranges = cdiv(ntiles, VB_GV_WAVES);
    if (nranges > max_ranges) nranges = max_ranges;
    if (nranges < 1) nranges = 1;
    VirtGvArgs a{wg_gnp, L->g_poolV, L->wpack, L->batch, Gv, cstride, N, C, ngroups, nranges};
    const size_t lds = (size_t)VB_GV_CH * RM_BYTES;
    ProfScope ps(K_VIRT_BWD_GV, st);
    if (bf) hipLaunchKernelGGL((virt_bwd_gv_kernel<true>), dim3(ngroups * nranges), dim3(64 * VB_GV_WAVES), lds, st, a);
    else hipLaunchKernelGGL((virt_bwd_gv_kernel<false>), dim3(ngroups * nranges), dim3(64 * VB_GV_WAVES), lds, st, a);
  }
  if ((rc = check_launch("virt_bwd_gv_kernel"))) return rc;
  WgradBatch bb(L->wg_slab, st, bf, WG_SLABS / 2, WG_SLABS / 2);
  VirtBwd2Args A;
  A.f = make_virt_args(L);
  A.g_x_out = L->g_x_out; A.g_poolX = L->g_poolX; A.Gv = Gv;
  A.g_x = L->g_x; A.g_A = L->g_A; A.g_Bc = L->g_Bc; A.g_Zp = L->g_Zp;
  A.gA_part = gA_part; A.gx_part = gx_part; A.wg_v = wg_v; A.cstride = cstride;
  A.cons_scratch = gx_part + (size_t)256 * VB_FINE_TILES * (NGF - 1) * 16 * 4;
  A.ld_v0 = 2 * H + 1 + C;
  A.d_wxv2 = g[FASTEGNN_P_CRV2_W]; A.d_wxx2 = g[FASTEGNN_P_CVV2_W];
  A.d_wvr = g[FASTEGNN_P_VIRT0_W] + 2 * H;
  A.d_attw = g[FASTEGNN_P_ATTV_W]; A.d_attb = g[FASTEGNN_P_ATTV_B];
  A.NGF = NGF;
  int grid = ntiles < 256 ? ntiles : 256;
  if ((rc = bb.add_slabs(g[FASTEGNN_P_CRV0_W], H, 0, 1, g[FASTEGNN_P_CRV0_B], grid, &A.slab_x))) return rc;
  if ((rc = bb.add_slabs(g[FASTEGNN_P_CVV0_W], H, 0, 1, g[FASTEGNN_P_CVV0_B], grid, &A.slab_X))) return rc;
  if ((rc = bb.add_slabs(g[FASTEGNN_P_VIRT2_W], H, 0, 1, g[FASTEGNN_P_VIRT2_B], grid, &A.slab_v2))) return rc;
  A.slab = bb.tab.slab; A.slab_b = bb.tab.slab_b;
  static const int ring_want = getenv("FE_VB_RING") ? atoi(getenv("FE_VB_RING")) : 54;
  const int imgb = bf ? RM_BYTES : (GM_VIRT_BWD == GM_F16 ? rm_lds_bytes<GM_F16>() : RM_BYTES);
  A.ringA = ring_want / 10; A.ringB = ring_want % 10; A.nbank = 1;
  if (A.ringA < 2 || A.ringA > VB_MAXRING) A.ringA = 3;
  if (A.ringB < 2 || A.ringB > VB_MAXRING) A.ringB = 3;
  while (vb_lds_floats(C, A.ringA, A.ringB, 1, imgb) * sizeof(float) > 160 * 1024 && A.ringB > 2) --A.ringB;
  while (vb_lds_floats(C, A.ringA, A.ringB, 1, imgb) * sizeof(float) > 160 * 1024 && A.ringA > 2) --A.ringA;
  while (A.nbank < VB_MAXBANK && vb_lds_floats(C, A.ringA, A.ringB, A.nbank + 1, imgb) * sizeof(float) <= 160 * 1024) ++A.nbank;
  const size_t lds = vb_lds_floats(C, A.ringA, A.ringB, A.nbank, imgb) * sizeof(float);
  FE_REQUIRE(lds <= 160 * 1024, "virt_backward: LDS budget exceeded");
  {
    ProfScope ps(K_VIRT_BWD, st);
    const dim3 g3(grid), b3(64 * VB_WAVES);
    if (bf) { if (att) hipLaunchKernelGGL((virt_bwd_pc_kernel<true, true>), g3, b3, lds, st, A); else hipLaunchKernelGGL((virt_bwd_pc_kernel<true, false>), g3, b3, lds, st, A); }
    else { if (att) hipLaunchKernelGGL((virt_bwd_pc_kernel<false, true>), g3, b3, lds, st, A); else hipLaunchKernelGGL((virt_bwd_pc_kernel<false, false>), g3, b3, lds, st, A); }
  }
  if ((rc = check_launch("virt_bwd_pc_kernel"))) return rc;
  if (NGF > 1) {
    hipLaunchKernelGGL(virt_bwd_combine_kernel, dim3(grid * VB_FINE_TILES), dim3(256), 0, st, L->g_A, L->g_x, gA_part, gx_part, N, NGF - 1, grid);
    if ((rc = check_launch("virt_bwd_combine_kernel"))) return rc;
  }
  if (!rf) {
    const int ld_n0 = 2 * H + H * C + L->na;
    if ((rc = bb.add(wg_gnp, H, wg_v, H, N, g[FASTEGNN_P_NODE0_W], ld_n0, 2 * H, C, nullptr, C, 0, (long)cstride, 1))) return rc;
  }
  return bb.finish();
}

int virt_backward(const fastegnn_layer_t *L, hipStream_t st, WgradBatch *shared) {
  const bool egnn = has(L, FASTEGNN_F_EGNN), rf = has(L, FASTEGNN_F_RF);
  FE_REQUIRE(L->h && L->A && L->x && L->vel && L->aggm && L->npre && L->batch && L->wpack && (!egnn || L->aggx),
             "virt_backward: null saved buffer");
  FE_REQUIRE(L->g_h_out && L->g_x_out && L->g_h && L->g_x && L->g_A && L->g_aggm && L->g_aggx && L->g_svel && L->wg_node &&
                 L->grads && L->wg_slab,
             "virt_backward: null gradient buffer");
  FE_REQUIRE(egnn ? L->C == 0
                  : (L->Bc && L->Z && (rf || L->g_poolV) && L->g_poolX && L->g_Bc && L->g_Zp && L->wg_virt && L->C >= 1 && L->C <= 64),
             "virt_backward: virtual buffers null or virtual_channels outside [1,64] (0 with FASTEGNN_F_EGNN)");
  const int N = L->N, C = L->C;
  if (C > 0) {
    (void)hipMemsetAsync(L->g_Bc, 0, (size_t)L->B * C * H * sizeof(float), st);
    (void)hipMemsetAsync(L->g_Zp, 0, (size_t)L->B * 3 * C * sizeof(float), st);
  }
  if (N == 0) return check_launch("virt_backward(memset)");
  const bool bf = has(L, FASTEGNN_F_BF16);
  float *const *g = L->grads;
  FE_REQUIRE(!has(L, FASTEGNN_F_ATTENTION) || C == 0 || (g[FASTEGNN_P_ATTV_W] && g[FASTEGNN_P_ATTV_B]), "virt_backward: attention grads null");
  FE_REQUIRE(!has(L, FASTEGNN_F_GRAVITY) || L->g_sgrav, "virt_backward: g_sgrav null");
  float *wg_t3 = L->wg_node, *wg_gnp = L->wg_node + (size_t)N * H;
  const int ntiles = cdiv(N, 16);
  int rc;
  {
    VirtNodeArgs a{L->g_h_out, L->npre, L->g_x_out, L->vel, L->aggx, L->wpack, wg_t3, wg_gnp, L->g_h, L->g_aggm, L->g_aggx,
                   L->g_svel, L->g_sgrav, N, L->flags, C, {L->gravity[0], L->gravity[1], L->gravity[2]}, L->act_param};
    int grid = cdiv(ntiles, VB_NODE_WAVES);
    if (grid > 256) grid = 256;
    ProfScope ps(K_VIRT_BWD_NODE, st);
    if (bf) hipLaunchKernelGGL((virt_bwd_node_kernel<true>), dim3(grid), dim3(64 * VB_NODE_WAVES), 3 * IMG3 * sizeof(float), st, a);
    else hipLaunchKernelGGL((virt_bwd_node_kernel<false>), dim3(grid), dim3(64 * VB_NODE_WAVES), 3 * IMG3 * sizeof(float), st, a);
  }
  if ((rc = check_launch("virt_bwd_node_kernel"))) return rc;
  if (C == 0) {
    (void)hipMemcpyAsync(L->g_x, L->g_x_out, (size_t)N * 3 * sizeof(float), hipMemcpyDeviceToDevice, st);
    (void)hipMemsetAsync(L->g_A, 0, (size_t)N * H * sizeof(float), st);
    if ((rc = check_launch("virt_backward(C = 0)"))) return rc;
  } else if ((rc = virt_backward_channels(L, st, wg_gnp))) {
    return rc;
  }
  if (rf) return FASTEGNN_OK;
  WgradBatch local(L->wg_slab, st);
  WgradBatch &wb = shared ? *shared : local;
  wb.round = bf;
  const int ld_n0 = 2 * H + H * C + L->na;
  if ((rc = wb.add(L->g_h_out, H, wg_t3, H, N, g[FASTEGNN_P_NODE2_W], H, 0, 1, g[FASTEGNN_P_NODE2_B]))) return rc;
  if ((rc = wb.add(wg_gnp, H, L->h, H, N, g[FASTEGNN_P_NODE0_W], ld_n0, 0, 1, g[FASTEGNN_P_NODE0_B]))) return rc;
  if ((rc = wb.add(wg_gnp, H, L->aggm, H, N, g[FASTEGNN_P_NODE0_W], ld_n0, H, 1, nullptr))) return rc;
  if (!shared && (rc = wb.finish())) return rc;
  if (L->na > 0) {
    if ((rc = launch_wgrad_small(wg_gnp, H, L->node_attr, L->na, L->na, N, g[FASTEGNN_P_NODE0_W], ld_n0, 2 * H + H * C, st))) return rc;
    if (L->g_node_attr)
      if ((rc = launch_dgrad_small(wg_gnp, N, L->na, L->params[FASTEGNN_P_NODE0_W], ld_n0, 2 * H + H * C, L->g_node_attr, 1, st))) return rc;
  }
  return FASTEGNN_OK;
}

}

#ifdef FE_STAMP
extern "C" int fastegnn_debug_read_vb2_stamps(unsigned long long *out, int reset) {
  if (hipMemcpyFromSymbol(out, HIP_SYMBOL(fe::g_vb2_stamps), sizeof(unsigned long long) * 32) != hipSuccess) return -1;
  if (reset) {
    unsigned long long z[32] = {0};
    (void)hipMemcpyToSymbol(HIP_SYMBOL(fe::g_vb2_stamps), z, sizeof(z));
  }
  return 0;
}
#endif

extern "C" int fastegnn_spin_timeouts(int reset) {
  int n = -1;
  if (hipMemcpyFromSymbol(&n, HIP_SYMBOL(fe::g_vbs_timeouts), sizeof(int)) != hipSuccess) return -1;
  if (reset) {
    const int z = 0;
    (void)hipMemcpyToSymbol(HIP_SYMBOL(fe::g_vbs_timeouts), &z, sizeof(int));
  }
  return n;
}
#ifdef FE_VBS_WATCHDOG
extern "C" int fastegnn_debug_read_vbs_dog(int *out, int reset) {
  if (hipMemcpyFromSymbol(out, HIP_SYMBOL(fe::g_vbs_dog), sizeof(int) * 64) != hipSuccess) return -1;
  if (reset) {
    int z[64] = {0};
    (void)hipMemcpyToSymbol(HIP_SYMBOL(fe::g_vbs_dog), z, sizeof(z));
  }
  return 0;
}
#endif
```

### fastegnn_amd/csrc/virt_fwd.h

```cpp
#pragma once
#include "stages.h"

namespace fe {

constexpr int VIRT_FWD_IMG_FLOATS = 5 * IMG3;
constexpr int VIRT_FWD_PAIR_STAGE = 4 * 4096;
constexpr int VIRT_FWD_IMG_FLOATS_PAIR = 3 * IMG3 + VIRT_FWD_PAIR_STAGE;
inline size_t virt_fwd_lds_bytes(int C, bool pair = false) {
  return (size_t)((pair ? VIRT_FWD_IMG_FLOATS_PAIR : VIRT_FWD_IMG_FLOATS) + VV_COUNT * H + 2 * (C * H + ((3 * C + 3) & ~3)) + 4) * sizeof(float);
}
template <int MODE, bool PAIR = false>
__global__ __launch_bounds__(64 * VIRT_WAVES) void virt_fwd_kernel(VirtArgs a) {
  static_assert(!PAIR || MODE == GM_F16, "the two-waves-per-tile walk is built for the f16x2 images");
  constexpr int TPS = PAIR ? VIRT_WAVES / 2 : VIRT_WAVES;
  extern __shared__ __attribute__((aligned(16))) float lds[];
  const int C = a.C;
  float *img = lds;
  unsigned *stage = reinterpret_cast<unsigned *>(lds) + 3 * IMG3;
  float *vec = lds + (PAIR ? VIRT_FWD_IMG_FLOATS_PAIR : VIRT_FWD_IMG_FLOATS);
  float *poolV_l = vec + VV_COUNT * H;
  float *poolX_l = poolV_l + C * H;
  float *Bc_l = poolX_l + ((3 * C + 3) & ~3);
  float *Z_l = Bc_l + C * H;
#ifdef VF_SPLIT_BARRIER
  int *ctl = reinterpret_cast<int *>(Z_l + ((3 * C + 3) & ~3));
  if (threadIdx.x < 4) ctl[threadIdx.x] = 0;
  int vf_steps = 0;
  auto vf_signal = [&](int k) {
    __builtin_amdgcn_fence(__ATOMIC_RELEASE, "workgroup");
    if (lane_id() == 0) atomicAdd(&ctl[k], 1);
  };
  auto vf_wait = [&](int k, int need) {
    while (__atomic_load_n(&ctl[k], __ATOMIC_RELAXED) < need) __builtin_amdgcn_s_sleep(1);
    __builtin_amdgcn_fence(__ATOMIC_ACQUIRE, "workgroup");
  };
#endif
  load_images_x3(reinterpret_cast<unsigned *>(img), wpack_x3(a.wpack, C, I_V2), 3);
  virt_load_vecs(vec, a);
  for (int i = threadIdx.x; i < C * H + 3 * C; i += blockDim.x) poolV_l[i] = 0.f;
  __syncthreads();
  const int l = lane_id(), j = l & 15, q = l >> 4, wv = wave_id();
  const int ntiles = (a.N + 15) >> 4;
  const int t_lo = (int)((long)blockIdx.x * ntiles / gridDim.x), t_hi = (int)((long)(blockIdx.x + 1) * ntiles / gridDim.x);
  const float invC = C > 0 ? 1.0f / (float)C : 0.f;
  const bool clamp_aggx = a.flags & FASTEGNN_F_EGNN;
  const bool rf = a.flags & FASTEGNN_F_RF;
  int cur = -1;
  VF_T0()
  auto flush_pools = [&]() {
    if (!rf)
      for (int i = threadIdx.x; i < C * H; i += blockDim.x) {
        atomicAdd(&a.poolV[(size_t)cur * C * H + i], poolV_l[i]);
        poolV_l[i] = 0.f;
      }
    for (int i = threadIdx.x; i < 3 * C; i += blockDim.x) {
      atomicAdd(&a.poolX[(size_t)cur * 3 * C + i], poolX_l[i]);
      poolX_l[i] = 0.f;
    }
  };
  static_assert(2048 == 4 * 64 * VIRT_WAVES, "one part of a split image per pass of the stage copy");
  constexpr int STG = MODE == GM_F16 ? 2 : 3;
  u32x4 pre_w[PAIR ? 2 * STG : STG];
  auto fetch_w3c = [&](int c) {
    if constexpr (PAIR) {
#pragma unroll
      for (int g = 0; g < 2; ++g) {
        const int cc = min(2 * c + g, C - 1);
        const u32x4 *src = reinterpret_cast<const u32x4 *>(wpack_x3(a.wpack, C, img_w3c(cc)));
#pragma unroll
        for (int i = 0; i < STG; ++i) pre_w[g * STG + i] = src[threadIdx.x + i * 64 * VIRT_WAVES];
      }
    } else {
      const u32x4 *src = reinterpret_cast<const u32x4 *>(wpack_x3(a.wpack, C, img_w3c(c)));
#pragma unroll
      for (int i = 0; i < STG; ++i) pre_w[i] = src[threadIdx.x + i * 64 * VIRT_WAVES];
    }
  };
  auto commit_w3c = [&](int slot) {
    if constexpr (PAIR) {
#pragma unroll
      for (int g = 0; g < 2; ++g) {
        u32x4 *dst = reinterpret_cast<u32x4 *>(stage + (2 * slot + g) * 4096);
#pragma unroll
        for (int i = 0; i < STG; ++i) dst[threadIdx.x + i * 64 * VIRT_WAVES] = pre_w[g * STG + i];
      }
    } else {
      u32x4 *dst = reinterpret_cast<u32x4 *>(stage + slot * IMG3);
#pragma unroll
      for (int i = 0; i < STG; ++i) dst[threadIdx.x + i * 64 * VIRT_WAVES] = pre_w[i];
    }
  };
  const int grp = PAIR ? wv >> 2 : 0;
  for (int tb = t_lo; tb < t_hi; tb += TPS) {
    const bool split = !PAIR && t_hi - tb == 1 && C >= VIRT_WAVES;
    const bool own = PAIR ? grp == 0 : (!split || wv == 0);
    const int n0 = tb * 16, nend = min(a.N, min(t_hi, tb + TPS) * 16);
    const int bfirst = a.batch[n0], blast = a.batch[nend - 1];
    const bool fast = bfirst == blast;
    const bool staged = C > 0 && !rf && !split;
    if (staged) fetch_w3c(0);
    if (fast && bfirst != cur) {
      __syncthreads();
      if (cur >= 0) flush_pools();
      cur = bfirst;
      for (int i = threadIdx.x; i < C * H; i += blockDim.x) Bc_l[i] = a.Bc[(size_t)cur * C * H + i];
      for (int i = threadIdx.x; i < 3 * C; i += blockDim.x) Z_l[i] = a.Z[(size_t)cur * 3 * C + i];
      __syncthreads();
    }
    const int nb = split ? n0 : n0 + (PAIR ? (wv & 3) : wv) * 16;
    const int nvalid = max(0, min(16, nend - nb));
    const bool active = nvalid > 0;
    const int n = nb + j;
    const bool valid = n < nend;
    const int nc = valid ? n : nend - 1;
    const int b = a.batch[nc];
    Vec Ai;
    float xi[3] = {0.f, 0.f, 0.f};
    if (active) {
      Ai = vload_row(a.A + (size_t)nc * H, q);
      xi[0] = a.x[(size_t)nc * 3]; xi[1] = a.x[(size_t)nc * 3 + 1]; xi[2] = a.x[(size_t)nc * 3 + 2];
    }
    float transv[3] = {0.f, 0.f, 0.f};
    Vec nodeacc = own ? vload_vec(vec + VV_B3 * H, q) : vzero();
    if (staged) {
      __syncthreads();
      commit_w3c(0);
#ifdef VF_SPLIT_BARRIER
      vf_signal(0);
#endif
      if ((PAIR ? (C + 1) / 2 : C) > 1) fetch_w3c(1);
    }
    const int n_it = PAIR ? (C + 1) / 2 : (split ? (C - wv + VIRT_WAVES - 1) / VIRT_WAVES : C);
    VF_T(8)
    for (int it = 0; it < n_it; ++it) {
      const int c = PAIR ? 2 * it + grp : (split ? wv + it * VIRT_WAVES : it);
      const bool chan = !PAIR || c < C;
#if defined(VF_SPLIT_BARRIER)
      static_assert(!PAIR, "VF_SPLIT_BARRIER is a lever of the one-wave-per-tile walk");
      if (staged) {
        const int sl = c & 1, s1 = sl ^ 1, per0 = (C + 1) >> 1, per1 = C >> 1;
        if (c + 1 < C) {
          vf_wait(2 + s1, VIRT_WAVES * (vf_steps * (s1 ? per1 : per0) + ((c + 2 - s1) >> 1)));
          commit_w3c(s1);
          vf_signal(s1);
          if (c + 2 < C) fetch_w3c(c + 2);
        }
        vf_wait(sl, VIRT_WAVES * (vf_steps * (sl ? per1 : per0) + (c >> 1) + 1));
      }
#elif !defined(VF_DIAG_NOSTAGE)
      if (staged) {
        __syncthreads();
        if (it + 1 < n_it) {
          commit_w3c((it + 1) & 1);
          if (it + 2 < n_it) fetch_w3c(it + 2);
        }
      }
#endif
      VF_T(0)
      if (active && chan) {
        VirtFwdState<MODE> S;
        virt_tile_forward<MODE>(a, img, vec, Ai, xi, b, c, q, fast ? Bc_l : nullptr, fast ? Z_l : nullptr, S VF_TA);
        transv[0] -= S.vd[0] * S.sx;
        transv[1] -= S.vd[1] * S.sx;
        transv[2] -= S.vd[2] * S.sx;
        if (fast) {
          if (!rf) tile_sum_add(poolV_l + c * H, nvalid == 16 ? S.v : (valid ? S.v : vzero()), j, q);
          const float p0 = jsum_dpp(valid ? S.vd[0] * S.sX : 0.f), p1 = jsum_dpp(valid ? S.vd[1] * S.sX : 0.f),
                      p2 = jsum_dpp(valid ? S.vd[2] * S.sX : 0.f);
          if (l < 3) atomicAdd(&poolX_l[l * C + c], l == 0 ? p0 : (l == 1 ? p1 : p2));
        } else {
          const int g_lo = __builtin_amdgcn_readlane(b, 0), g_hi = __builtin_amdgcn_readlane(b, nvalid - 1);
          for (int g = g_lo; g <= g_hi; ++g) {
            const bool in_g = valid && b == g;
            if (!rf) tile_sum_add(a.poolV + ((size_t)g * C + c) * H, in_g ? S.v : vzero(), j, q);
            const float p0 = jsum_dpp(in_g ? S.vd[0] * S.sX : 0.f), p1 = jsum_dpp(in_g ? S.vd[1] * S.sX : 0.f),
                        p2 = jsum_dpp(in_g ? S.vd[2] * S.sX : 0.f);
            if (l < 3) atomicAdd(&a.poolX[((size_t)g * 3 + l) * C + c], l == 0 ? p0 : (l == 1 ? p1 : p2));
          }
        }
        VF_T(6)
        if (!rf) {
#ifdef VF_DIAG_NODE_IMG0
          gemm_op<MODE>(img, 0, S.vs, nodeacc);
#elif defined(VF_DIAG_NONODE)
          if (S.vs.p[0][0][0] == 0x12345678u) nodeacc = S.v;
#else
          if (split) gemm_op<MODE>(wpack_x3(a.wpack, C, img_w3c(c)), 0, S.vs, nodeacc);
          else if constexpr (PAIR) gemm64_f2<false>(stage, S.vs, nodeacc, (2 * (it & 1) + (int)(threadIdx.x >> 8)) * 1024);
          else gemm_op<MODE>(stage + (c & 1) * IMG3, 0, S.vs, nodeacc);
#endif
        }
        VF_T(7)
      }
#ifdef VF_SPLIT_BARRIER
      if (staged) vf_signal(2 + (c & 1));
#endif
    }
#ifdef VF_SPLIT_BARRIER
    if (staged) ++vf_steps;
#endif
    if constexpr (PAIR) {
      float *comb = lds + 3 * IMG3;
      const int co = ((wv & 3) * 16 + j) * TS;
      __syncthreads();
      if (grp == 1 && active) {
#pragma unroll
        for (int t = 0; t < 4; ++t) *reinterpret_cast<f32x4 *>(&comb[co + 16 * t + 4 * q]) = nodeacc.t[t];
        if (q == 0) *reinterpret_cast<f32x4 *>(&comb[co + H]) = f32x4{transv[0], transv[1], transv[2], 0.f};
      }
      __syncthreads();
      if (grp == 0 && active) {
#pragma unroll
        for (int t = 0; t < 4; ++t) nodeacc.t[t] += *reinterpret_cast<const f32x4 *>(&comb[co + 16 * t + 4 * q]);
#pragma unroll
        for (int k = 0; k < 3; ++k) transv[k] += comb[co + H + k];
      }
    }
    if (split) {
      float *comb = reinterpret_cast<float *>(stage);
      __syncthreads();
      for (int i = threadIdx.x; i < 16 * TS; i += blockDim.x) comb[i] = 0.f;
      __syncthreads();
#pragma unroll
      for (int t = 0; t < 4; ++t)
#pragma unroll
        for (int r = 0; r < 4; ++r) atomicAdd(&comb[j * TS + 16 * t + 4 * q + r], nodeacc.t[t][r]);
      if (q == 0) {
#pragma unroll
        for (int k = 0; k < 3; ++k) atomicAdd(&comb[j * TS + H + k], transv[k]);
      }
      __syncthreads();
      if (own) {
#pragma unroll
        for (int t = 0; t < 4; ++t) nodeacc.t[t] = *reinterpret_cast<const f32x4 *>(comb + j * TS + 16 * t + 4 * q);
#pragma unroll
        for (int k = 0; k < 3; ++k) transv[k] = comb[j * TS + H + k];
      }
      __syncthreads();
    }
    if (active && rf && own) {
      if (valid) vstore_row(a.h_out + (size_t)n * H, q, vload_row(a.h + (size_t)nc * H, q));
    }
    if (!rf) {
      const bool mine = active && own;
      auto stage_image = [&](int id) {
        const u32x4 *src = reinterpret_cast<const u32x4 *>(wpack_x3(a.wpack, C, id));
        u32x4 tmp[STG];
#pragma unroll
        for (int i = 0; i < STG; ++i) tmp[i] = src[threadIdx.x + i * 64 * VIRT_WAVES];
        __syncthreads();
        u32x4 *dst = reinterpret_cast<u32x4 *>(stage);
#pragma unroll
        for (int i = 0; i < STG; ++i) dst[threadIdx.x + i * 64 * VIRT_WAVES] = tmp[i];
        __syncthreads();
      };
      Vec hv = vzero();
      stage_image(I_W3A);
      if (mine) {
        hv = vload_row(a.h + (size_t)nc * H, q);
        gemm_i<MODE>(stage, 0, hv, nodeacc);
      }
      stage_image(I_W3B);
      if (mine) {
        gemm_i<MODE>(stage, 0, vload_row(a.aggm + (size_t)nc * H, q), nodeacc);
        if (a.na > 0) {
          const int ld = 2 * H + H * C + a.na;
          for (int k = 0; k < a.na; ++k) {
            const float av = a.node_attr[(size_t)nc * a.na + k];
#pragma unroll
            for (int t = 0; t < 4; ++t)
#pragma unroll
              for (int r = 0; r < 4; ++r)
                nodeacc.t[t][r] += av * a.N0W[(size_t)(16 * t + 4 * q + r) * ld + 2 * H + H * C + k];
          }
        }
        if (valid) vstore_row(a.npre + (size_t)n * H, q, nodeacc);
      }
      stage_image(I_W4);
      if (mine) {
        Vec out = vload_vec(vec + VV_B4 * H, q);
        gemm_i<MODE>(stage, 0, vsilu(nodeacc FE_ACT(a)), out);
        if (a.flags & FASTEGNN_F_RESIDUAL) vadd(out, hv);
        if (valid) vstore_row(a.h_out + (size_t)n * H, q, out);
      }
    }
    VF_T(9)
    if (active && own) {
      if (valid) {
        if (q == 0) {
          const float sv = a.svel[n];
          const float sg = (a.flags & FASTEGNN_F_GRAVITY) ? a.sgrav[n] : 0.f;
#pragma unroll
          for (int k = 0; k < 3; ++k) {
            float ax = a.aggx[(size_t)n * 3 + k];
            if (clamp_aggx) ax = ax > 100.f ? 100.f : (ax < -100.f ? -100.f : ax);
            a.x_out[(size_t)n * 3 + k] = xi[k] + ax + transv[k] * invC + sv * a.vel[(size_t)n * 3 + k] + sg * a.g[k];
          }
        }
      }
    }
  }
  __syncthreads();
  if (cur >= 0) flush_pools();
  VF_T(10)
  VF_TEND()
}

}
```

### fastegnn_amd/csrc/virt_fwd_pair.hip

```cpp
#include "virt_fwd.h"

namespace fe {

void launch_virt_fwd_pair(const VirtArgs &a, int grid, size_t lds, hipStream_t st) {
  if constexpr (GM_VIRT_FWD == GM_F16)
    hipLaunchKernelGGL((virt_fwd_kernel<GM_F16, true>), dim3(grid), dim3(64 * VIRT_WAVES), lds, st, a);
  else
    (void)a, (void)grid, (void)lds, (void)st;
}

}
```

### fastegnn_amd/model.py

```python
from __future__ import annotations

import ctypes as C
import math
import os
from typing import Dict, List, Optional

import torch
from torch import nn

from . import _lib as K

H = K.H


class E_GCL_vel(nn.Module):

    def __init__(self, hidden_nf, node_attr_nf, edge_attr_nf, virtual_channels, act_fn, attention, tanh, gravity):
        super().__init__()
        Hn, Cn = hidden_nf, virtual_channels
        self.edge_mlp = nn.Sequential(nn.Linear(2 * Hn + 1 + edge_attr_nf, Hn), act_fn, nn.Linear(Hn, Hn), act_fn)
        self.edge_mlp_virtual = nn.Sequential(nn.Linear(2 * Hn + 1 + Cn, Hn), act_fn, nn.Linear(Hn, Hn), act_fn)
        if attention:
            self.att_mlp = nn.Sequential(nn.Linear(Hn, 1), nn.Sigmoid())
            self.att_mlp_virtual = nn.Sequential(nn.Linear(Hn, 1), nn.Sigmoid())
# ... 259 lines not shown

class _Spec:

    def __init__(self, model: "FastEGNN", deterministic: Optional[bool] = None):
        self.C = model.virtual_channels
        self.n_layers = model.n_layers
        self.ea = model.edge_attr_nf
        self.na = model.node_attr_nf
        self.nf = model.node_feat_nf
        flags = 0
        flags |= K.F_ATTENTION if model.attention else 0
        flags |= K.F_NORMALIZE if model.normalize else 0
        flags |= K.F_TANH if model.tanh else 0
        flags |= K.F_RESIDUAL if model.residual else 0
        flags |= K.F_GRAVITY if model.gravity is not None else 0
        flags |= K.F_BF16 if getattr(model, "mlp_dtype", torch.float32) == torch.bfloat16 else 0
        det = getattr(model, "deterministic", False) if deterministic is None else deterministic
        flags |= K.F_DETERMINISTIC if det else 0
        self.act_kind, self.act_param = getattr(model, "_act", (K.ACT_SILU, 0.0))
        flags |= self.act_kind << K.F_ACT_SHIFT
        self.flags = flags | model._extra_flags
        self.wide = False
        self.guard = None
        self.gravity = [float(v) for v in model.gravity] if model.gravity is not None else [0.0, 0.0, 0.0]
        self.names = ["virtual_node_feat", "embedding_in.weight", "embedding_in.bias"]
        self.layer_slots: List[List[Optional[int]]] = []
        pidx = model._param_index
        for i in range(model.n_layers):
            slots = []
            for suffix in K.PARAM_SLOTS:
                key = f"gcl_{i}.{suffix}"
                if key in pidx:
                    slots.append(len(self.names))
                    self.names.append(key)
                else:
                    slots.append(None)
            self.layer_slots.append(slots)


def _new_layer(spec: _Spec, N: int, B: int, graph: SortedGraph) -> K.LayerT:
    L = K.LayerT()
    L.N, L.B, L.C, L.ea, L.na, L.flags = N, B, spec.C, spec.ea, spec.na, spec.flags
    L.gravity = (C.c_float * 3)(*spec.gravity)
    L.epsilon = 1e-8
    L.act_param = getattr(spec, "act_param", 0.0)
    L.graph = graph.struct()
    return L


_HIDDEN_OUT = ("edge_mlp.0", "edge_mlp.2", "edge_mlp_virtual.0", "edge_mlp_virtual.2", "coord_mlp_r.0",
               "coord_mlp_r_virtual.0", "coord_mlp_v_virtual.0", "coord_mlp_vel.0", "gravity_mlp.0", "node_mlp.0",
               "node_mlp.2", "node_mlp_virtual.0", "node_mlp_virtual.2", "embedding_in")


def _pad_layout(name: str, shape, h: int, C_: int, rf: bool):
    shape = tuple(shape)
    if name == "virtual_node_feat":
        return h, shape[2], H, [], (1, H, shape[2])
    mod, kind = name.rsplit(".", 1)
    mod = mod.split(".", 1)[1] if mod.startswith("gcl_") else mod
    if kind == "bias":
        if mod in _HIDDEN_OUT:
            return 1, shape[0], 1, [h], (H,)
        return 1, shape[0], 1, [], shape
    if mod in ("edge_mlp.0", "edge_mlp_virtual.0", "node_mlp_virtual.0"):
        blocks = [h, h]
    elif mod == "node_mlp.0":
        blocks = [h, h, h * C_]
    elif mod == "embedding_in" or (rf and mod == "coord_mlp_vel.0"):
        blocks = []
    else:
        blocks = [h]
    rows, cols = shape
    rows_dst = H if mod in _HIDDEN_OUT else rows
    cols_dst = cols + sum(b // h * (H - h) for b in blocks)
    return rows, cols, rows_dst, blocks, (rows_dst, cols_dst)


def _activation_kind(act_fn: nn.Module):
    if isinstance(act_fn, nn.SiLU):
        return K.ACT_SILU, 0.0
    if isinstance(act_fn, nn.ReLU):
        return K.ACT_RELU, 0.0
    if isinstance(act_fn, nn.LeakyReLU):
        return K.ACT_LEAKY_RELU, float(act_fn.negative_slope)
    if isinstance(act_fn, nn.Tanh):
        return K.ACT_TANH, 0.0
    if isinstance(act_fn, nn.Sigmoid):
        return K.ACT_SIGMOID, 0.0
    if isinstance(act_fn, nn.ELU):
        return K.ACT_ELU, float(act_fn.alpha)
    if isinstance(act_fn, nn.GELU) and getattr(act_fn, "approximate", "none") == "none":
        return K.ACT_GELU, 0.0
    if isinstance(act_fn, nn.Softplus) and float(act_fn.threshold) == 20.0:
        return K.ACT_SOFTPLUS, float(act_fn.beta)
    raise NotImplementedError("fastegnn_amd: act_fn must be one of SiLU, ReLU, LeakyReLU, Tanh, Sigmoid, ELU, GELU "
                              f"(exact) or Softplus(threshold=20); got {act_fn!r}")


class _PadParams(torch.autograd.Function):

    @staticmethod
    def _table(layouts, narrow, wide):
        tab = (K.PadDesc * len(layouts))()
        for d, lay, a, b in zip(tab, layouts, narrow, wide):
            rows, cols, rows_dst, blocks = lay[:4]
            d.lead = lay[5] if len(lay) > 5 else 0
            d.src, d.dst = a.data_ptr(), b.data_ptr()
            d.rows, d.cols, d.rows_dst = rows, cols, rows_dst
            d.cols_dst = b.numel() // max(rows_dst, 1)
            d.nblk = len(blocks)
            for i, blk in enumerate(blocks):
                d.blk[i] = blk
        return tab

    @staticmethod
    def forward(ctx, names, h, C_, rf, *params):
        lib = K.lib()
        dev = params[0].device
        layouts = [(rf(n, p.shape, h) if callable(rf) else _pad_layout(n, p.shape, h, C_, rf)) for n, p in zip(names, params)]
        sizes = [(math.prod(l[4]) + 3) // 4 * 4 for l in layouts]
        flat = torch.empty(sum(sizes), device=dev, dtype=torch.float32)
        outs, off = [], 0
        for l, sz in zip(layouts, sizes):
            outs.append(flat[off:off + math.prod(l[4])].view(l[4]))
            off += sz
        src = [p.detach().contiguous().float() for p in params]
        tab = _PadParams._table(layouts, src, outs)
        K.check(lib.fastegnn_pad_params(tab, len(layouts), h, 0, _stream(dev)), "fastegnn_pad_params")
        ctx.layouts, ctx.h, ctx.shapes = layouts, h, [p.shape for p in params]
        return tuple(outs)

    @staticmethod
    def backward(ctx, *gouts):
        lib = K.lib()
        idx = [i for i, g in enumerate(gouts) if g is not None]
        grads = [None] * len(gouts)
        if idx:
            dev = gouts[idx[0]].device
            wide = [gouts[i].contiguous().float() for i in idx]
            sizes = [(math.prod(ctx.shapes[i]) + 3) // 4 * 4 for i in idx]
            flat = torch.empty(sum(sizes), device=dev, dtype=torch.float32)
            narrow, off = [], 0
            for i, sz in zip(idx, sizes):
                narrow.append(flat[off:off + math.prod(ctx.shapes[i])].view(ctx.shapes[i]))
                off += sz
            tab = _PadParams._table([ctx.layouts[i] for i in idx], narrow, wide)
            K.check(lib.fastegnn_pad_params(tab, len(idx), ctx.h, 1, _stream(dev)), "fastegnn_pad_params")
            for i, g in zip(idx, narrow):
                grads[i] = g
        return (None, None, None, None, *grads)


class _FastEGNNFunction(torch.autograd.Function):

    @staticmethod
    def forward(ctx, spec: _Spec, graph: SortedGraph, batch32, gptr, edge_attr, node_attr,
                node_feat, node_loc, node_vel, loc_mean, *params):
        lib = K.lib(act=spec.act_kind != K.ACT_SILU, wide=spec.wide)
        ctx.wide = spec.wide
        ctx.guard = getattr(spec, "guard", None)
        ea_sorted = graph.permute(edge_attr.detach() if edge_attr is not None else None)
        node_attr = node_attr.detach().contiguous().float() if node_attr is not None else None
        dev = node_loc.device
        st = _stream(dev)
        N, B, Cn = node_loc.size(0), loc_mean.size(0), spec.C
        f32 = dict(dtype=torch.float32, device=dev)
        params = [p.detach() for p in params]
        for p in params:
            if p.dtype != torch.float32 or not p.is_contiguous() or p.data_ptr() % 16:
                raise RuntimeError("fastegnn_amd: parameters must be contiguous, 16-byte aligned fp32 tensors")
        node_feat, node_loc, node_vel, loc_mean = (t.detach().contiguous().float()
                                                   for t in (node_feat, node_loc, node_vel, loc_mean))
        h = torch.empty(N, H, **f32)
        K.check(lib.fastegnn_embed_forward(K.ptr(node_feat), N, spec.nf, K.ptr(params[1]), K.ptr(params[2]),
                                           K.ptr(h), st), "fastegnn_embed_forward")
        HvT = torch.empty(B, Cn, H, **f32)
        K.check(lib.fastegnn_virtual_init(K.ptr(params[0]), B, Cn, K.ptr(HvT), st), "fastegnn_virtual_init")
        x, Z = node_loc, loc_mean
        saved = []
        nwp = (lib.fastegnn_wpack_floats(Cn) + 3) // 4 * 4
        wpack_all = torch.empty(spec.n_layers, nwp, **f32)
        tabs = [_PtrTable([params[s] if s is not None else None for s in spec.layer_slots[i]]) for i in range(spec.n_layers)]
        packs = (C.POINTER(K.LayerT) * spec.n_layers)()
        keep = []
        for i in range(spec.n_layers):
            Lp = _new_layer(spec, N, B, graph)
            _fill(Lp, params=tabs[i].addr(), wpack=wpack_all[i])
            keep.append(Lp)
            packs[i] = C.pointer(Lp)
        K.check(lib.fastegnn_pack_weights_all(packs, spec.n_layers, st), "fastegnn_pack_weights_all")
        for i in range(spec.n_layers):
            tab = tabs[i]
            b = dict(h=h, x=x, Z=Z, HvT=HvT, wpack=wpack_all[i])
            b.update(_carve(dev, dict(
                P=(N, H), QX=(N, K.QX_LD), A=(N, H), svel=(N,), sgrav=(N,), xsum=(B, 4),
                Bc=(B, Cn, H), aggm=(N, H), npre=(N, H), poolV=(B, Cn, H))))
            b.update(_carve(dev, dict(aggx=(N, 3), poolX=(B, 3, Cn))))
            b.update(h_out=torch.empty(N, H, **f32), x_out=torch.empty(N, 3, **f32),
                     Z_out=torch.empty(B, 3, Cn, **f32), HvT_out=torch.empty(B, Cn, H, **f32))
            L = _new_layer(spec, N, B, graph)
            L.flags |= K.F_WPACK_READY
            _fill(L, batch=batch32, gptr=gptr, vel=node_vel, params=tab.addr(), **b)
            L.QX_src = b["QX"].data_ptr()
            if ea_sorted is not None:
                L.ea_sorted = ea_sorted.data_ptr()
            if node_attr is not None:
                L.node_attr = node_attr.data_ptr()
            K.check(lib.fastegnn_layer_forward(C.byref(L), st), f"fastegnn_layer_forward[{i}]")
            saved.append(b)
            h, x, Z, HvT = b["h_out"], b["x_out"], b["Z_out"], b["HvT_out"]
            for k in ("aggx", "poolX", "h_out", "x_out", "Z_out", "HvT_out"):
                del b[k]
        ctx.spec, ctx.graph, ctx.saved = spec, graph, saved
        ctx.misc = (batch32, gptr, ea_sorted, node_attr, node_feat, node_vel, params)
        return x, Z

    @staticmethod
    @torch.autograd.function.once_differentiable
    def backward(ctx, g_loc, g_vloc):
        lib = K.lib(act=ctx.spec.act_kind != K.ACT_SILU, wide=ctx.wide)
        spec, graph, saved = ctx.spec, ctx.graph, ctx.saved
        guard = ctx.guard
        if guard is not None:
            guard.poll("FastEGNN", ctx.misc[-1])
        if saved is None or any(b is None for b in saved):
            raise RuntimeError("fastegnn_amd: backward through the graph a second time: the saved stage products are "
                               "freed layer by layer during the first backward (retain_graph is not supported)")
        batch32, gptr, ea_sorted, node_attr, node_feat, node_vel, params = ctx.misc
        dev = node_vel.device
        st = _stream(dev)
        N, B, Cn, E = node_vel.size(0), saved[0]["Z"].size(0), spec.C, graph.E
        f32 = dict(dtype=torch.float32, device=dev)
        sizes = [(p.numel() + 3) // 4 * 4 for p in params]
        flat = torch.zeros(sum(sizes), **f32)
        grads, off = [], 0
        for p, s in zip(params, sizes):
            grads.append(flat[off:off + p.numel()].view_as(p))
            off += s
        g_h = torch.zeros(N, H, **f32)
        g_x = (g_loc if g_loc is not None else torch.zeros(N, 3, **f32)).contiguous().float()
        g_Z = (g_vloc if g_vloc is not None else torch.zeros(B, 3, Cn, **f32)).contiguous().float()
        g_HvT = torch.zeros(B, Cn, H, **f32)
        g_vel = torch.zeros(N, 3, **f32)
        want_ea = ctx.needs_input_grad[4] and ea_sorted is not None and E > 0
        want_na = ctx.needs_input_grad[5] and node_attr is not None
        g_ea_sorted = torch.zeros(E, spec.ea, **f32) if want_ea else None
        g_na = torch.zeros(N, spec.na, **f32) if want_na else None
        scratch = _carve(dev, dict(
            g_poolV=(B, Cn, H), g_poolX=(B, 3, Cn), g_Bc=(B, Cn, H), g_Zp=(B, 3, Cn), g_xbar=(B, 4),
            g_A=(N, H), g_P=(N, H), g_aggm=(N, H), g_aggx=(N, 3), g_svel=(N,), g_sgrav=(N,),
            g_QXe=(max(E, 1) if spec.flags & K.F_DETERMINISTIC else 1, K.QX_LD), g_QX_src=(N, K.QX_LD), g_xrow=(N, 3),
            wg_edge=(lib.fastegnn_wg_edge_floats(E),), wg_virt=(lib.fastegnn_wg_virt_floats_for(N, Cn, spec.flags),),
            wg_node=(lib.fastegnn_wg_node_floats(N, B, Cn),),
            wg_slab=(lib.fastegnn_wg_slab_floats(),)))
        for i in reversed(range(spec.n_layers)):
            b = saved[i]
            ptab = _PtrTable([params[s] if s is not None else None for s in spec.layer_slots[i]])
            gtab = _PtrTable([grads[s] if s is not None else None for s in spec.layer_slots[i]])
            L = _new_layer(spec, N, B, graph)
            out = dict(g_h=torch.empty(N, H, **f32), g_x=torch.empty(N, 3, **f32),
                       g_Z=torch.empty(B, 3, Cn, **f32), g_HvT=torch.empty(B, Cn, H, **f32))
            _fill(L, batch=batch32, gptr=gptr, vel=node_vel, params=ptab.addr(), grads=gtab.addr(),
                  g_h_out=g_h, g_x_out=g_x, g_Z_out=g_Z, g_HvT_out=g_HvT, g_vel=g_vel, **b, **out, **scratch)
            L.QX_src = b["QX"].data_ptr()
            L.g_QX = scratch["g_QX_src"].data_ptr()
            if ea_sorted is not None:
                L.ea_sorted = ea_sorted.data_ptr()
            if node_attr is not None:
                L.node_attr = node_attr.data_ptr()
            if g_ea_sorted is not None:
                L.g_ea_sorted = g_ea_sorted.data_ptr()
            if g_na is not None:
                L.g_node_attr = g_na.data_ptr()
            K.check(lib.fastegnn_layer_backward(C.byref(L), st), f"fastegnn_layer_backward[{i}]")
            g_h, g_x, g_Z, g_HvT = out["g_h"], out["g_x"], out["g_Z"], out["g_HvT"]
            saved[i] = None
        K.check(lib.fastegnn_virtual_init_backward(K.ptr(g_HvT), B, Cn, K.ptr(grads[0]), st),
                "fastegnn_virtual_init_backward")
        g_nf = torch.empty_like(node_feat) if ctx.needs_input_grad[6] else None
        g_ea = None
        if g_ea_sorted is not None:
            g_ea = torch.empty_like(g_ea_sorted)
            g_ea.index_copy_(0, graph.perm[:E].long(), g_ea_sorted)
        K.check(lib.fastegnn_embed_backward(K.ptr(node_feat), K.ptr(g_h), N, spec.nf, K.ptr(params[1]),
                                            K.ptr(grads[1]), K.ptr(grads[2]), K.ptr(g_nf), st),
                "fastegnn_embed_backward")
        if guard is not None:
            guard.zero_if_flagged(lib, flat)
        last = spec.n_layers - 1
        for s_, suffix in zip(spec.layer_slots[last], K.PARAM_SLOTS):
            if s_ is not None and suffix.startswith(("node_mlp.", "node_mlp_virtual.")) and not (spec.flags & K.F_RF):
                grads[s_] = None
        return (None, None, None, None, g_ea, g_na, g_nf, g_x, g_vel, g_Z, *grads)


class FastEGNN(nn.Module):

    _layer_cls = E_GCL_vel
    _extra_flags = 0

    def __init__(self, node_feat_nf, node_attr_nf, edge_attr_nf, hidden_nf, virtual_channels, device='cpu',
                 act_fn=nn.SiLU(), n_layers=4, residual=True, attention=False, normalize=False, tanh=False,
                 gravity=None, *, mlp_dtype=torch.float32):
        super().__init__()
        if mlp_dtype not in (torch.float32, torch.bfloat16):
            raise ValueError("fastegnn_amd: mlp_dtype must be torch.float32 or torch.bfloat16")
        self.mlp_dtype = mlp_dtype
        assert virtual_channels > 0, f'Channels of virtual node must greater than 0 (got {virtual_channels})'
        self._wide = hidden_nf > H or virtual_channels > 64 or edge_attr_nf > 7 or node_feat_nf > 8
        if not 1 <= hidden_nf <= 256:
            raise NotImplementedError(f"fastegnn_amd: hidden_nf must be at most 256 in this build (got {hidden_nf})")
        if self._wide and mlp_dtype != torch.float32:
            raise NotImplementedError("fastegnn_amd: hidden_nf > 64, virtual_channels > 64, edge_attr_nf > 7 or node_feat_nf > 8 run on "
                                      "the unfused wide path, which is built for fp32 operands only")
        self._act = _activation_kind(act_fn)
        if self._act[0] in (K.ACT_SIGMOID, K.ACT_SOFTPLUS) and hidden_nf < H:
            raise NotImplementedError("fastegnn_amd: hidden_nf < 64 runs zero-padded, which needs act_fn(0) = 0")
        if self._act[0] != K.ACT_SILU and mlp_dtype != torch.float32:
            raise NotImplementedError("fastegnn_amd: the bf16 operand mode is built for SiLU only")
        self.hidden_nf = hidden_nf
        self.device = device
        self.n_layers = n_layers
        self.virtual_channels = virtual_channels
        self.node_feat_nf, self.node_attr_nf, self.edge_attr_nf = node_feat_nf, node_attr_nf, edge_attr_nf
        self.residual, self.attention, self.normalize, self.tanh = residual, attention, normalize, tanh
        self.gravity = list(gravity) if gravity is not None else None
        self.virtual_node_feat = nn.Parameter(data=torch.randn(size=(1, hidden_nf, virtual_channels)),
                                              requires_grad=True)
        self.embedding_in = nn.Linear(node_feat_nf, self.hidden_nf)
        for i in range(n_layers):
            self.add_module("gcl_%d" % i, self._layer_cls(hidden_nf, node_attr_nf, edge_attr_nf, virtual_channels, act_fn,
                                                          attention, tanh, gravity))
        self._graph_cache: Dict[tuple, SortedGraph] = {}
        self.cache_graphs = True
        self._range = RangeGuard()
        self._deterministic = K.deterministic_default()
        self._spec = None
        self._spec_det = None
        self._plist = None
        self.to(self.device)

    @property
    def _param_index(self):
        return dict(self.named_parameters())

    @property
    def deterministic(self) -> bool:
        if self._deterministic is None:
            return self.mlp_dtype == torch.bfloat16
        return self._deterministic

    @deterministic.setter
    def deterministic(self, value):
        self._deterministic = None if value is None else bool(value)
        self._spec = None
        self._spec_det = None
        self._graph_cache = {}

    SMALL_GRAPH_EDGES = 512

    def deterministic_for(self, n_edges: int) -> bool:
        if self._deterministic is None and n_edges <= self.SMALL_GRAPH_EDGES:
            return True
        return self.deterministic

    def sorted_graph(self, edge_index: torch.Tensor, n_nodes: int, deterministic: Optional[bool] = None) -> SortedGraph:
        det = self.deterministic_for(edge_index.size(1)) if deterministic is None else deterministic
        key = (edge_index.data_ptr(), edge_index.size(1), edge_index._version, n_nodes, n_nodes, 0, det)
        g = self._graph_cache.get(key) if self.cache_graphs else None
        if g is None:
            g = SortedGraph(edge_index, n_nodes, csc=det)
            if self.cache_graphs:
                if len(self._graph_cache) >= 8:
                    self._graph_cache.pop(next(iter(self._graph_cache)))
                g._keepalive = edge_index
                self._graph_cache[key] = g
        return g

    def forward(self, node_feat, node_loc, node_vel, edge_index, data_batch, loc_mean, edge_attr=None,
                node_attr=None):
        if not node_loc.is_cuda:
            raise RuntimeError("fastegnn_amd.FastEGNN runs on a gfx950 GPU only (no CPU fallback): move the model "
                               "and its inputs to 'cuda'")
        if (edge_attr.size(1) if edge_attr is not None else 0) != self.edge_attr_nf:
            raise ValueError("edge_attr width does not match edge_attr_nf")
        if (node_attr.size(1) if node_attr is not None else 0) != self.node_attr_nf:
            raise ValueError("node_attr width does not match node_attr_nf")
        if self._wide:
            from . import wide
            if isinstance(edge_index, SortedGraph):
                raise TypeError("fastegnn_amd: the wide path (hidden_nf > 64) takes edge_index as the reference does, an int64 [2, E] tensor")
            if _DEBUG_CHECKS:
                _check_indices(edge_index, data_batch, node_loc.size(0), loc_mean.size(0))
            if edge_attr is not None and edge_attr.size(1) == 0:
                edge_attr = None
            return wide.forward(self, node_feat, node_loc, node_vel, edge_index, data_batch, loc_mean, edge_attr, node_attr)
        dev = node_loc.device
        N, B = node_loc.size(0), loc_mean.size(0)
        if self._spec is None:
            self._spec = _Spec(self)
            pidx = self._param_index
            self._plist = [pidx[n] for n in self._spec.names]
        graph = edge_index if isinstance(edge_index, SortedGraph) else self.sorted_graph(edge_index, N)
        spec = self._spec
        if graph.cscptr is not None and not spec.flags & K.F_DETERMINISTIC:
            if getattr(self, "_spec_det", None) is None:
                self._spec_det = _Spec(self, deterministic=True)
            spec = self._spec_det
        elif graph.cscptr is None and spec.flags & K.F_DETERMINISTIC:
            raise ValueError("fastegnn_amd: deterministic=True needs a SortedGraph built with csc=True")
        lib = K.lib()
        if data_batch.dtype != torch.int64:
            data_batch = data_batch.long()
        if _DEBUG_CHECKS:
            _check_indices(edge_index, data_batch, N, B)
        batch32 = torch.empty(N, dtype=torch.int32, device=dev)
# ... 30 lines not shown
```

Baseline: 96.81 graphs/s.

## Skip dead final-layer node and virtual-feature updates in forward and backward

The model returns only coordinates (x, Z), so the last layer's h_out and HvT_out are never consumed. The final layer now skips the node MLP, the poolV accumulation and the graph-post feature MLP in the forward pass. In the backward pass it runs coordinate-only kernels and NODE=false template variants in place of the node and virtual-feature gradient work. This removes GEMMs, LDS traffic and weight-gradient batches for one of four layers, at the cost of many new code paths and null-pointer contracts. It is gated by an env var and on by default.

Measured after the change: 100.8 graphs/s (median of 6 runs). +4.1%, better.

```diff
diff --git a/fastegnn_amd/csrc/layer_bwd.hip b/fastegnn_amd/csrc/layer_bwd.hip
--- a/fastegnn_amd/csrc/layer_bwd.hip
+++ b/fastegnn_amd/csrc/layer_bwd.hip
@@ -76,7 +76,27 @@
   }
 }
 
+__global__ __launch_bounds__(256) void graph_post_bwd_coords_kernel(const float *xsum, const float *g_Z_out, float *g_Z, float *g_poolX,
+                                                                    float *g_HvT, int B, int C) {
+  for (int i = blockIdx.x * blockDim.x + threadIdx.x; i < B * 3 * C; i += gridDim.x * blockDim.x) {
+    const int b = i / (3 * C);
+    const float g = g_Z_out[i];
+    g_Z[i] = g;
+    g_poolX[i] = g / fmaxf(xsum[b * 4 + 3], 1.f);
+  }
+  for (int i = blockIdx.x * blockDim.x + threadIdx.x; i < B * C * H; i += gridDim.x * blockDim.x) g_HvT[i] = 0.f;
+}
+
 int graph_post_backward(const fastegnn_layer_t *L, hipStream_t st, WgradBatch *shared) {
+  if (!L->g_HvT_out && !has(L, FASTEGNN_F_RF)) {
+    FE_REQUIRE(!L->g_h_out, "graph_post_backward: g_HvT_out is null and g_h_out is not (both null: no gradient for h / Hv; otherwise neither)");
+    FE_REQUIRE(L->xsum && L->g_Z_out && L->g_Z && L->g_HvT && L->g_poolX, "graph_post_backward: null buffer");
+    int grid = cdiv((long)L->B * L->C * H, 256);
+    if (grid > 256) grid = 256;
+    if (grid < 1) grid = 1;
+    { ProfScope _ps_graph_post_bwd_kernel(K_GRAPH_POST_BWD, st); hipLaunchKernelGGL(graph_post_bwd_coords_kernel, dim3(grid), dim3(256), 0, st, L->xsum, L->g_Z_out, L->g_Z, L->g_poolX, L->g_HvT, L->B, L->C); }
+    return check_launch("graph_post_bwd_coords_kernel");
+  }
   FE_REQUIRE(L->xsum && L->HvT && L->poolV && L->g_Z_out && L->g_HvT_out && L->g_Z && L->g_HvT && L->g_poolV &&
                  L->g_poolX && L->wg_node && L->grads && L->wpack,
              "graph_post_backward: null buffer");
diff --git a/fastegnn_amd/csrc/layer_fwd.hip b/fastegnn_amd/csrc/layer_fwd.hip
--- a/fastegnn_amd/csrc/layer_fwd.hip
+++ b/fastegnn_amd/csrc/layer_fwd.hip
@@ -350,14 +350,16 @@
 
 int virt_forward(const fastegnn_layer_t *L, hipStream_t st) {
   const bool egnn = has(L, FASTEGNN_F_EGNN);
-  FE_REQUIRE(L->h && L->A && L->x && L->vel && L->aggm && L->aggx && L->svel && L->npre && L->h_out && L->x_out &&
+  const bool node = egnn || has(L, FASTEGNN_F_RF) || L->h_out;
+  FE_REQUIRE(node || !L->HvT_out, "virt_forward: h_out is null and HvT_out is not (both null: no node update; otherwise neither)");
+  FE_REQUIRE(L->h && L->A && L->x && L->vel && L->aggm && L->aggx && L->svel && (!node || (L->npre && L->h_out)) && L->x_out &&
                  L->batch && L->wpack,
              "virt_forward: null buffer");
-  FE_REQUIRE(egnn ? L->C == 0 : (L->Bc && L->Z && L->poolV && L->poolX && L->C >= 1 && L->C <= 64),
+  FE_REQUIRE(egnn ? L->C == 0 : (L->Bc && L->Z && (!node || L->poolV) && L->poolX && L->C >= 1 && L->C <= 64),
              "virt_forward: virtual_channels must be in [1,64] (0 with FASTEGNN_F_EGNN) and the virtual buffers non-null");
   FE_REQUIRE(L->na == 0 || L->node_attr, "virt_forward: node_attr null");
   if (L->C > 0) {
-    (void)hipMemsetAsync(L->poolV, 0, (size_t)L->B * L->C * H * sizeof(float), st);
+    if (node) (void)hipMemsetAsync(L->poolV, 0, (size_t)L->B * L->C * H * sizeof(float), st);
     (void)hipMemsetAsync(L->poolX, 0, (size_t)L->B * 3 * L->C * sizeof(float), st);
   }
   if (L->N == 0) return check_launch("virt_forward(memset)");
@@ -370,7 +372,12 @@
   {
     ProfScope _ps_virt_fwd_kernel(K_VIRT_FWD, st);
     const size_t lds = virt_fwd_lds_bytes(L->C, pair);
-    if (has(L, FASTEGNN_F_BF16)) hipLaunchKernelGGL(virt_fwd_kernel<GM_BF16>, dim3(grid), dim3(64 * VIRT_WAVES), lds, st, a);
+    if (!node) {
+      if (has(L, FASTEGNN_F_BF16)) hipLaunchKernelGGL((virt_fwd_kernel<GM_BF16, false, false>), dim3(grid), dim3(64 * VIRT_WAVES), lds, st, a);
+      else if (pair) launch_virt_fwd_pair_nonode(a, grid, lds, st);
+      else hipLaunchKernelGGL((virt_fwd_kernel<GM_VIRT_FWD, false, false>), dim3(grid), dim3(64 * VIRT_WAVES), lds, st, a);
+    }
+    else if (has(L, FASTEGNN_F_BF16)) hipLaunchKernelGGL(virt_fwd_kernel<GM_BF16>, dim3(grid), dim3(64 * VIRT_WAVES), lds, st, a);
     else if (pair) launch_virt_fwd_pair(a, grid, lds, st);
     else hipLaunchKernelGGL(virt_fwd_kernel<GM_VIRT_FWD>, dim3(grid), dim3(64 * VIRT_WAVES), lds, st, a);
   }
@@ -414,7 +421,23 @@
     if (valid) vstore_row(a.HvT_out + (size_t)m * H, q, out);
   }
 }
+__global__ __launch_bounds__(256) void graph_post_fwd_coords_kernel(const float *xsum, const float *Z, const float *poolX, float *Z_out,
+                                                                    int B, int C) {
+  for (int i = blockIdx.x * blockDim.x + threadIdx.x; i < B * 3 * C; i += gridDim.x * blockDim.x) {
+    const int b = i / (3 * C);
+    Z_out[i] = Z[i] + poolX[i] / fmaxf(xsum[b * 4 + 3], 1.f);
+  }
+}
 int graph_post_forward(const fastegnn_layer_t *L, hipStream_t st) {
+  if (!L->HvT_out && !has(L, FASTEGNN_F_RF)) {
+    FE_REQUIRE(!L->h_out, "graph_post_forward: HvT_out is null and h_out is not (both null: no node update; otherwise neither)");
+    FE_REQUIRE(L->xsum && L->Z && L->poolX && L->Z_out, "graph_post_forward: null buffer");
+    int grid = cdiv((long)L->B * 3 * L->C, 256);
+    if (grid > 256) grid = 256;
+    if (grid < 1) grid = 1;
+    { ProfScope _ps_graph_post_fwd_kernel(K_GRAPH_POST_FWD, st); hipLaunchKernelGGL(graph_post_fwd_coords_kernel, dim3(grid), dim3(256), 0, st, L->xsum, L->Z, L->poolX, L->Z_out, L->B, L->C); }
+    return check_launch("graph_post_fwd_coords_kernel");
+  }
   FE_REQUIRE(L->xsum && L->Z && L->HvT && L->poolV && L->poolX && L->Z_out && L->HvT_out && L->wpack,
              "graph_post_forward: null buffer");
   GraphPostArgs a{L->xsum, L->Z, L->HvT, L->poolV, L->poolX, L->wpack, L->params[FASTEGNN_P_NODEV0_B],
diff --git a/fastegnn_amd/csrc/stages.h b/fastegnn_amd/csrc/stages.h
--- a/fastegnn_amd/csrc/stages.h
+++ b/fastegnn_amd/csrc/stages.h
@@ -353,6 +353,7 @@
   return a;
 }
 void launch_virt_fwd_pair(const VirtArgs &a, int grid, size_t lds, hipStream_t st);
+void launch_virt_fwd_pair_nonode(const VirtArgs &a, int grid, size_t lds, hipStream_t st);
 inline size_t virt_lds_bytes(int C, int n_img, int waves = VIRT_WAVES) {
   return (size_t)(n_img * IMG + 16 * H + waves * 16 * TS + C * H + 4 * C) * sizeof(float);
 }
diff --git a/fastegnn_amd/csrc/virt_bwd.hip b/fastegnn_amd/csrc/virt_bwd.hip
--- a/fastegnn_amd/csrc/virt_bwd.hip
+++ b/fastegnn_amd/csrc/virt_bwd.hip
@@ -95,6 +95,30 @@
   }
 }
 
+__global__ __launch_bounds__(256) void virt_bwd_node_skip_kernel(const float *g_x_out, const float *vel, float *g_h, float *g_aggm,
+                                                                 float *g_aggx, float *g_svel, float *g_sgrav, int N, int flags,
+                                                                 float g0, float g1, float g2) {
+  const size_t i = (size_t)blockIdx.x * blockDim.x + threadIdx.x;
+  if (i >= (size_t)N * (H / 4)) return;
+  const f32x4 z = {0.f, 0.f, 0.f, 0.f};
+  reinterpret_cast<f32x4 *>(g_h)[i] = z;
+  reinterpret_cast<f32x4 *>(g_aggm)[i] = z;
+  if ((i & (H / 4 - 1)) == 0) {
+    const size_t n = i / (H / 4);
+    const float g[3] = {g0, g1, g2};
+    float sv = 0.f, sg = 0.f;
+#pragma unroll
+    for (int k = 0; k < 3; ++k) {
+      const float gxn = g_x_out[n * 3 + k];
+      g_aggx[n * 3 + k] = gxn;
+      sv += gxn * vel[n * 3 + k];
+      sg += gxn * g[k];
+    }
+    g_svel[n] = sv;
+    if (flags & FASTEGNN_F_GRAVITY) g_sgrav[n] = sg;
+  }
+}
+
 struct VirtGvArgs {
   const float *g_np, *g_poolV, *wpack;
   const int32_t *batch;
@@ -847,7 +871,7 @@
 #endif
 constexpr int VBS_SPIN_LIMIT = 1 << 23;
 __device__ int g_vbs_timeouts = 0;
-template <bool ATT>
+template <bool ATT, bool NODE = true>
 __global__ __launch_bounds__(64 * VB_WAVES) void virt_bwd_cs_kernel(VirtCsArgs A) {
   constexpr int SM = GM_F16;
   typedef typename OperandOf<SM>::type SOp;
@@ -897,13 +921,15 @@
   const int nblk = max(1, (nt + A.block / 2) / A.block);
   const int BT = (nt + nblk - 1) / nblk;
   const int nphase = nblk * C;
-  if (wv == 0) stage_w3(0);
-  if (wv == 1 && nphase > 1) stage_w3(1);
+  if constexpr (NODE) {
+    if (wv == 0) stage_w3(0);
+    if (wv == 1 && nphase > 1) stage_w3(1);
+  }
   __syncthreads();
   if (threadIdx.x < 2 && (int)threadIdx.x < nphase) ctrl[VBSC_READY + threadIdx.x] = threadIdx.x + 1;
   __syncthreads();
   constexpr bool FIVEP = FE_VBS_5P != 0;
-  const bool consumer = wv == VB_CONS_X || wv == VB_CONS_XX || (FIVEP && wv == VB_CONS_V2);
+  const bool consumer = wv == VB_CONS_X || wv == VB_CONS_XX || (FIVEP && NODE && wv == VB_CONS_V2);
   const int total = nt * C;
   const int cur = a.batch[t_lo * 16];
   const bool tanh_on = a.flags & FASTEGNN_F_TANH;
@@ -1010,10 +1036,11 @@
       int since_w = 0;
       int *drainedA = ctrl + VBSC_DRAINED + VB_MAXRING, *drainedB = ctrl + VBSC_DRAINED + 2 * VB_MAXRING;
 #ifdef FE_VBS_SWAP
-      const bool doV2 = FIVEP ? wv == VB_CONS_V2 : wv == VB_CONS_XX, doW = wv == VB_CONS_XX;
+      const bool doV2n = FIVEP ? wv == VB_CONS_V2 : wv == VB_CONS_XX, doWn = wv == VB_CONS_XX;
 #else
-      const bool doV2 = wv == VB_CONS_XX, doW = FIVEP ? wv == VB_CONS_V2 : wv == VB_CONS_XX;
-#endif
+      const bool doV2n = wv == VB_CONS_XX, doWn = FIVEP ? wv == VB_CONS_V2 : wv == VB_CONS_XX;
+#endif
+      const bool doV2 = NODE ? doV2n : true, doW = NODE && doWn;
       auto flush_w = [&](WgAcc32 &acc, float ig, float it, int slot, bool have, float *dst, bool add) {
 #pragma unroll
         for (int bo = 0; bo < 2; ++bo)
@@ -1253,28 +1280,34 @@
         }
       }
       VB2_T(6)
-      const Vec gnp = vb_mask(vload_u(A.g_np, offN), valid);
+      Vec gnp = vzero();
+      if constexpr (NODE) gnp = vb_mask(vload_u(A.g_np, offN), valid);
       {
         int tk = 0;
         if (l == 0) tk = atomicAdd(&ctrl[VBSC_HEAD + 0], 1);
         tk = __builtin_amdgcn_readfirstlane(tk);
         const int sl = tk % A.ringA, round = tk / A.ringA;
         VBS_SPIN(4, vb_ld(&ctrl[VBSC_DRAINED + 0 * VB_MAXRING + sl]) != round, 2);
-        VBS_SPIN(5, vb_ld(&ctrl[VBSC_DRAINED + 1 * VB_MAXRING + sl]) != round, 2);
+        if constexpr (NODE) VBS_SPIN(5, vb_ld(&ctrl[VBSC_DRAINED + 1 * VB_MAXRING + sl]) != round, 2);
         __builtin_amdgcn_fence(__ATOMIC_ACQUIRE, "workgroup", "local");
         float *slot = ringA + sl * VBS_SLOT_A;
         vb_tile_store(slot, j, q, g_ux);
         vb_tile_store(slot + VB_TILE, j, q, g_uX);
         vb_tile_store(slot + 2 * VB_TILE, j, q, valid ? v : vzero());
-        vb_tile_store(slot + 3 * VB_TILE, j, q, gnp);
-        if (l == 0) ctrl[VBSC_SLOTCH + sl] = c | (nb << 8) | (blk << 20);
+        if constexpr (NODE) {
+          vb_tile_store(slot + 3 * VB_TILE, j, q, gnp);
+          if (l == 0) ctrl[VBSC_SLOTCH + sl] = c | (nb << 8) | (blk << 20);
+        }
         __builtin_amdgcn_fence(__ATOMIC_RELEASE, "workgroup", "local");
         if (l == 0) vb_st(&ctrl[VBSC_FILLED + sl], round + 1);
         asm volatile("" ::: "memory");
       }
       VB2_T(7)
-      Vec g_v = vb_mask(vload_u(A.g_poolV, offB), valid);
-      gemm64_f2_scaled(w3 + (ph & 1) * VBS_W3_WORDS, vsplit2_scaled(gnp), g_v);
+      Vec g_v = vzero();
+      if constexpr (NODE) {
+        g_v = vb_mask(vload_u(A.g_poolV, offB), valid);
+        gemm64_f2_scaled(w3 + (ph & 1) * VBS_W3_WORDS, vsplit2_scaled(gnp), g_v);
+      }
       mmT(1, g_ux, g_v);
       mmT(2, g_uX, g_v);
       VB2_T(8)
@@ -1368,7 +1401,7 @@
         }
         if (l == 0) ctrl[VBSC_DONE + ph % VBS_NPH] = 0;
         if (ph + 2 < nphase) {
-          stage_w3(ph + 2);
+          if constexpr (NODE) stage_w3(ph + 2);
           asm volatile("" ::: "memory");
           if (l == 0) __hip_atomic_store(&ctrl[VBSC_READY + (ph + 2) % VBS_NPH], ph + 3, __ATOMIC_RELEASE, __HIP_MEMORY_SCOPE_WORKGROUP);
           asm volatile("" ::: "memory");
@@ -1426,12 +1459,12 @@
   return (N + WGV_PAD) * C * H + (size_t)256 * VB_FINE_TILES * (NGF - 1) * 16 * (H + 4) + (size_t)256 * 3 * IMG;
 }
 
-static int virt_backward_channels_cs(const fastegnn_layer_t *L, hipStream_t st, float *wg_gnp) {
+static int virt_backward_channels_cs(const fastegnn_layer_t *L, hipStream_t st, float *wg_gnp, bool node) {
   const int C = L->C;
   const bool att = has(L, FASTEGNN_F_ATTENTION);
   float *const *g = L->grads;
   const int grid = virt_cs_grid(L->N);
-  FE_REQUIRE(L->g_poolV, "virt_backward: g_poolV null");
+  FE_REQUIRE(!node || L->g_poolV, "virt_backward: g_poolV null");
   WgradBatch bb(L->wg_slab, st, false, WG_SLABS / 2, WG_SLABS / 2);
   VirtCsArgs A;
   A.f = make_virt_args(L);
@@ -1462,17 +1495,22 @@
   {
     ProfScope ps(K_VIRT_BWD, st);
     const dim3 g3(grid), b3(64 * VB_WAVES);
-    if (att) hipLaunchKernelGGL((virt_bwd_cs_kernel<true>), g3, b3, lds, st, A);
+    if (!node) {
+      if (att) hipLaunchKernelGGL((virt_bwd_cs_kernel<true, false>), g3, b3, lds, st, A);
+      else hipLaunchKernelGGL((virt_bwd_cs_kernel<false, false>), g3, b3, lds, st, A);
+    }
+    else if (att) hipLaunchKernelGGL((virt_bwd_cs_kernel<true>), g3, b3, lds, st, A);
     else hipLaunchKernelGGL((virt_bwd_cs_kernel<false>), g3, b3, lds, st, A);
   }
   if ((rc = check_launch("virt_bwd_cs_kernel"))) return rc;
+  if (!node) return bb.finish();
   const int ld_n0 = 2 * H + H * C + L->na;
   if ((rc = bb.add_slabs_ext(A.w_slab, g[FASTEGNN_P_NODE0_W], ld_n0, 2 * H, C, grid, C, 1))) return rc;
   return bb.finish();
 }
 
-static int virt_backward_channels(const fastegnn_layer_t *L, hipStream_t st, float *wg_gnp) {
-  if (virt_cs_applies(L->N, L->C, L->flags)) return virt_backward_channels_cs(L, st, wg_gnp);
+static int virt_backward_channels(const fastegnn_layer_t *L, hipStream_t st, float *wg_gnp, bool node) {
+  if (virt_cs_applies(L->N, L->C, L->flags)) return virt_backward_channels_cs(L, st, wg_gnp, node);
   const int N = L->N, C = L->C, ntiles = cdiv(N, 16);
   const bool bf = has(L, FASTEGNN_F_BF16), att = has(L, FASTEGNN_F_ATTENTION), rf = has(L, FASTEGNN_F_RF);
   float *const *g = L->grads;
@@ -1482,6 +1520,9 @@
   float *gA_part = Gv + cstride * C, *gx_part = gA_part + (size_t)256 * VB_FINE_TILES * (NGF - 1) * 16 * H;
   int rc;
   if (rf) {
+    (void)hipMemsetAsync(Gv, 0, cstride * C * sizeof(float), st);
+  } else if (!node) {
+    ProfScope ps(K_VIRT_BWD_GV, st);
     (void)hipMemsetAsync(Gv, 0, cstride * C * sizeof(float), st);
   } else {
     const int ngroups = cdiv(C, VB_GV_CH);
@@ -1534,7 +1575,7 @@
     hipLaunchKernelGGL(virt_bwd_combine_kernel, dim3(grid * VB_FINE_TILES), dim3(256), 0, st, L->g_A, L->g_x, gA_part, gx_part, N, NGF - 1, grid);
     if ((rc = check_launch("virt_bwd_combine_kernel"))) return rc;
   }
-  if (!rf) {
+  if (!rf && node) {
     const int ld_n0 = 2 * H + H * C + L->na;
     if ((rc = bb.add(wg_gnp, H, wg_v, H, N, g[FASTEGNN_P_NODE0_W], ld_n0, 2 * H, C, nullptr, C, 0, (long)cstride, 1))) return rc;
   }
@@ -1543,13 +1584,15 @@
 
 int virt_backward(const fastegnn_layer_t *L, hipStream_t st, WgradBatch *shared) {
   const bool egnn = has(L, FASTEGNN_F_EGNN), rf = has(L, FASTEGNN_F_RF);
-  FE_REQUIRE(L->h && L->A && L->x && L->vel && L->aggm && L->npre && L->batch && L->wpack && (!egnn || L->aggx),
+  const bool node = egnn || rf || L->g_h_out;
+  FE_REQUIRE(node || !L->g_HvT_out, "virt_backward: g_h_out is null and g_HvT_out is not (both null: no gradient for h / Hv; otherwise neither)");
+  FE_REQUIRE(L->h && L->A && L->x && L->vel && L->aggm && (!node || L->npre) && L->batch && L->wpack && (!egnn || L->aggx),
              "virt_backward: null saved buffer");
-  FE_REQUIRE(L->g_h_out && L->g_x_out && L->g_h && L->g_x && L->g_A && L->g_aggm && L->g_aggx && L->g_svel && L->wg_node &&
+  FE_REQUIRE((!node || L->g_h_out) && L->g_x_out && L->g_h && L->g_x && L->g_A && L->g_aggm && L->g_aggx && L->g_svel && L->wg_node &&
                  L->grads && L->wg_slab,
              "virt_backward: null gradient buffer");
   FE_REQUIRE(egnn ? L->C == 0
-                  : (L->Bc && L->Z && (rf || L->g_poolV) && L->g_poolX && L->g_Bc && L->g_Zp && L->wg_virt && L->C >= 1 && L->C <= 64),
+                  : (L->Bc && L->Z && (rf || !node || L->g_poolV) && L->g_poolX && L->g_Bc && L->g_Zp && L->wg_virt && L->C >= 1 && L->C <= 64),
              "virt_backward: virtual buffers null or virtual_channels outside [1,64] (0 with FASTEGNN_F_EGNN)");
   const int N = L->N, C = L->C;
   if (C > 0) {
@@ -1564,7 +1607,11 @@
   float *wg_t3 = L->wg_node, *wg_gnp = L->wg_node + (size_t)N * H;
   const int ntiles = cdiv(N, 16);
   int rc;
-  {
+  if (!node) {
+    ProfScope ps(K_VIRT_BWD_NODE, st);
+    hipLaunchKernelGGL(virt_bwd_node_skip_kernel, dim3(cdiv((long)N * (H / 4), 256)), dim3(256), 0, st, L->g_x_out, L->vel, L->g_h, L->g_aggm,
+                       L->g_aggx, L->g_svel, L->g_sgrav, N, L->flags, L->gravity[0], L->gravity[1], L->gravity[2]);
+  } else {
     VirtNodeArgs a{L->g_h_out, L->npre, L->g_x_out, L->vel, L->aggx, L->wpack, wg_t3, wg_gnp, L->g_h, L->g_aggm, L->g_aggx,
                    L->g_svel, L->g_sgrav, N, L->flags, C, {L->gravity[0], L->gravity[1], L->gravity[2]}, L->act_param};
     int grid = cdiv(ntiles, VB_NODE_WAVES);
@@ -1578,10 +1625,10 @@
     (void)hipMemcpyAsync(L->g_x, L->g_x_out, (size_t)N * 3 * sizeof(float), hipMemcpyDeviceToDevice, st);
     (void)hipMemsetAsync(L->g_A, 0, (size_t)N * H * sizeof(float), st);
     if ((rc = check_launch("virt_backward(C = 0)"))) return rc;
-  } else if ((rc = virt_backward_channels(L, st, wg_gnp))) {
+  } else if ((rc = virt_backward_channels(L, st, wg_gnp, node))) {
     return rc;
   }
-  if (rf) return FASTEGNN_OK;
+  if (rf || !node) return FASTEGNN_OK;
   WgradBatch local(L->wg_slab, st);
   WgradBatch &wb = shared ? *shared : local;
   wb.round = bf;
diff --git a/fastegnn_amd/csrc/virt_fwd.h b/fastegnn_amd/csrc/virt_fwd.h
--- a/fastegnn_amd/csrc/virt_fwd.h
+++ b/fastegnn_amd/csrc/virt_fwd.h
@@ -9,7 +9,7 @@
 inline size_t virt_fwd_lds_bytes(int C, bool pair = false) {
   return (size_t)((pair ? VIRT_FWD_IMG_FLOATS_PAIR : VIRT_FWD_IMG_FLOATS) + VV_COUNT * H + 2 * (C * H + ((3 * C + 3) & ~3)) + 4) * sizeof(float);
 }
-template <int MODE, bool PAIR = false>
+template <int MODE, bool PAIR = false, bool NODE = true>
 __global__ __launch_bounds__(64 * VIRT_WAVES) void virt_fwd_kernel(VirtArgs a) {
   static_assert(!PAIR || MODE == GM_F16, "the two-waves-per-tile walk is built for the f16x2 images");
   constexpr int TPS = PAIR ? VIRT_WAVES / 2 : VIRT_WAVES;
@@ -44,7 +44,7 @@
   const int t_lo = (int)((long)blockIdx.x * ntiles / gridDim.x), t_hi = (int)((long)(blockIdx.x + 1) * ntiles / gridDim.x);
   const float invC = C > 0 ? 1.0f / (float)C : 0.f;
   const bool clamp_aggx = a.flags & FASTEGNN_F_EGNN;
-  const bool rf = a.flags & FASTEGNN_F_RF;
+  const bool rf = !NODE || (a.flags & FASTEGNN_F_RF);
   int cur = -1;
   VF_T0()
   auto flush_pools = [&]() {
@@ -204,14 +204,18 @@
       const int co = ((wv & 3) * 16 + j) * TS;
       __syncthreads();
       if (grp == 1 && active) {
-#pragma unroll
-        for (int t = 0; t < 4; ++t) *reinterpret_cast<f32x4 *>(&comb[co + 16 * t + 4 * q]) = nodeacc.t[t];
+        if constexpr (NODE) {
+#pragma unroll
+          for (int t = 0; t < 4; ++t) *reinterpret_cast<f32x4 *>(&comb[co + 16 * t + 4 * q]) = nodeacc.t[t];
+        }
         if (q == 0) *reinterpret_cast<f32x4 *>(&comb[co + H]) = f32x4{transv[0], transv[1], transv[2], 0.f};
       }
       __syncthreads();
       if (grp == 0 && active) {
-#pragma unroll
-        for (int t = 0; t < 4; ++t) nodeacc.t[t] += *reinterpret_cast<const f32x4 *>(&comb[co + 16 * t + 4 * q]);
+        if constexpr (NODE) {
+#pragma unroll
+          for (int t = 0; t < 4; ++t) nodeacc.t[t] += *reinterpret_cast<const f32x4 *>(&comb[co + 16 * t + 4 * q]);
+        }
 #pragma unroll
         for (int k = 0; k < 3; ++k) transv[k] += comb[co + H + k];
       }
@@ -221,25 +225,31 @@
       __syncthreads();
       for (int i = threadIdx.x; i < 16 * TS; i += blockDim.x) comb[i] = 0.f;
       __syncthreads();
-#pragma unroll
-      for (int t = 0; t < 4; ++t)
-#pragma unroll
-        for (int r = 0; r < 4; ++r) atomicAdd(&comb[j * TS + 16 * t + 4 * q + r], nodeacc.t[t][r]);
+      if constexpr (NODE) {
+#pragma unroll
+        for (int t = 0; t < 4; ++t)
+#pragma unroll
+          for (int r = 0; r < 4; ++r) atomicAdd(&comb[j * TS + 16 * t + 4 * q + r], nodeacc.t[t][r]);
+      }
       if (q == 0) {
 #pragma unroll
         for (int k = 0; k < 3; ++k) atomicAdd(&comb[j * TS + H + k], transv[k]);
       }
       __syncthreads();
       if (own) {
-#pragma unroll
-        for (int t = 0; t < 4; ++t) nodeacc.t[t] = *reinterpret_cast<const f32x4 *>(comb + j * TS + 16 * t + 4 * q);
+        if constexpr (NODE) {
+#pragma unroll
+          for (int t = 0; t < 4; ++t) nodeacc.t[t] = *reinterpret_cast<const f32x4 *>(comb + j * TS + 16 * t + 4 * q);
+        }
 #pragma unroll
         for (int k = 0; k < 3; ++k) transv[k] = comb[j * TS + H + k];
       }
       __syncthreads();
     }
-    if (active && rf && own) {
-      if (valid) vstore_row(a.h_out + (size_t)n * H, q, vload_row(a.h + (size_t)nc * H, q));
+    if constexpr (NODE) {
+      if (active && rf && own) {
+        if (valid) vstore_row(a.h_out + (size_t)n * H, q, vload_row(a.h + (size_t)nc * H, q));
+      }
     }
     if (!rf) {
       const bool mine = active && own;
diff --git a/fastegnn_amd/csrc/virt_fwd_pair.hip b/fastegnn_amd/csrc/virt_fwd_pair.hip
--- a/fastegnn_amd/csrc/virt_fwd_pair.hip
+++ b/fastegnn_amd/csrc/virt_fwd_pair.hip
@@ -8,5 +8,11 @@
   else
     (void)a, (void)grid, (void)lds, (void)st;
 }
+void launch_virt_fwd_pair_nonode(const VirtArgs &a, int grid, size_t lds, hipStream_t st) {
+  if constexpr (GM_VIRT_FWD == GM_F16)
+    hipLaunchKernelGGL((virt_fwd_kernel<GM_F16, true, false>), dim3(grid), dim3(64 * VIRT_WAVES), lds, st, a);
+  else
+    (void)a, (void)grid, (void)lds, (void)st;
+}
 
 }
diff --git a/fastegnn_amd/model.py b/fastegnn_amd/model.py
--- a/fastegnn_amd/model.py
+++ b/fastegnn_amd/model.py
@@ -435,6 +435,10 @@
         return (None, None, None, None, *grads)
 
 
+def _skip_last_node_update(spec) -> bool:
+    return not (spec.flags & K.F_RF) and os.environ.get("FASTEGNN_KEEP_DEAD_NODE_UPDATE", "0") in ("", "0")
+
+
 class _FastEGNNFunction(torch.autograd.Function):
 
     @staticmethod
@@ -473,15 +477,21 @@
             keep.append(Lp)
             packs[i] = C.pointer(Lp)
         K.check(lib.fastegnn_pack_weights_all(packs, spec.n_layers, st), "fastegnn_pack_weights_all")
+        skip_last = _skip_last_node_update(spec)
         for i in range(spec.n_layers):
             tab = tabs[i]
+            dead = skip_last and i == spec.n_layers - 1
             b = dict(h=h, x=x, Z=Z, HvT=HvT, wpack=wpack_all[i])
-            b.update(_carve(dev, dict(
+            shapes = dict(
                 P=(N, H), QX=(N, K.QX_LD), A=(N, H), svel=(N,), sgrav=(N,), xsum=(B, 4),
-                Bc=(B, Cn, H), aggm=(N, H), npre=(N, H), poolV=(B, Cn, H))))
+                Bc=(B, Cn, H), aggm=(N, H), npre=(N, H), poolV=(B, Cn, H))
+            if dead:
+                del shapes["npre"], shapes["poolV"]
+            b.update(_carve(dev, shapes))
             b.update(_carve(dev, dict(aggx=(N, 3), poolX=(B, 3, Cn))))
-            b.update(h_out=torch.empty(N, H, **f32), x_out=torch.empty(N, 3, **f32),
-                     Z_out=torch.empty(B, 3, Cn, **f32), HvT_out=torch.empty(B, Cn, H, **f32))
+            b.update(x_out=torch.empty(N, 3, **f32), Z_out=torch.empty(B, 3, Cn, **f32))
+            if not dead:
+                b.update(h_out=torch.empty(N, H, **f32), HvT_out=torch.empty(B, Cn, H, **f32))
             L = _new_layer(spec, N, B, graph)
             L.flags |= K.F_WPACK_READY
             _fill(L, batch=batch32, gptr=gptr, vel=node_vel, params=tab.addr(), **b)
@@ -492,10 +502,11 @@
                 L.node_attr = node_attr.data_ptr()
             K.check(lib.fastegnn_layer_forward(C.byref(L), st), f"fastegnn_layer_forward[{i}]")
             saved.append(b)
-            h, x, Z, HvT = b["h_out"], b["x_out"], b["Z_out"], b["HvT_out"]
+            h, x, Z, HvT = b.get("h_out"), b["x_out"], b["Z_out"], b.get("HvT_out")
             for k in ("aggx", "poolX", "h_out", "x_out", "Z_out", "HvT_out"):
-                del b[k]
+                b.pop(k, None)
         ctx.spec, ctx.graph, ctx.saved = spec, graph, saved
+        ctx.skip_last = skip_last and spec.n_layers >= 1
         ctx.misc = (batch32, gptr, ea_sorted, node_attr, node_feat, node_vel, params)
         return x, Z
 
@@ -521,10 +532,11 @@
         for p, s in zip(params, sizes):
             grads.append(flat[off:off + p.numel()].view_as(p))
             off += s
-        g_h = torch.zeros(N, H, **f32)
+        skip_last = ctx.skip_last
+        g_h = None if skip_last else torch.zeros(N, H, **f32)
         g_x = (g_loc if g_loc is not None else torch.zeros(N, 3, **f32)).contiguous().float()
         g_Z = (g_vloc if g_vloc is not None else torch.zeros(B, 3, Cn, **f32)).contiguous().float()
-        g_HvT = torch.zeros(B, Cn, H, **f32)
+        g_HvT = None if skip_last else torch.zeros(B, Cn, H, **f32)
         g_vel = torch.zeros(N, 3, **f32)
         want_ea = ctx.needs_input_grad[4] and ea_sorted is not None and E > 0
         want_na = ctx.needs_input_grad[5] and node_attr is not None
@@ -544,8 +556,11 @@
             L = _new_layer(spec, N, B, graph)
             out = dict(g_h=torch.empty(N, H, **f32), g_x=torch.empty(N, 3, **f32),
                        g_Z=torch.empty(B, 3, Cn, **f32), g_HvT=torch.empty(B, Cn, H, **f32))
+            up = dict(g_x_out=g_x, g_Z_out=g_Z)
+            if g_h is not None:
+                up.update(g_h_out=g_h, g_HvT_out=g_HvT)
             _fill(L, batch=batch32, gptr=gptr, vel=node_vel, params=ptab.addr(), grads=gtab.addr(),
-                  g_h_out=g_h, g_x_out=g_x, g_Z_out=g_Z, g_HvT_out=g_HvT, g_vel=g_vel, **b, **out, **scratch)
+                  g_vel=g_vel, **up, **b, **out, **scratch)
             L.QX_src = b["QX"].data_ptr()
             L.g_QX = scratch["g_QX_src"].data_ptr()
             if ea_sorted is not None:
```
